# Banksylel/Restrictive-Hierarchical-Semantic-Segmentation

Measured on AMD Instinct MI355X. Metric: train images/sec (620x620, hier-HRNet-W48), higher is better.
Workload: dtype f32 (fp16x2 split on fp16 MFMA, 22-bit operands, fp32 accumulate; exact-fp32 MFMA on the small problems); 1 GPU; HRNet-W48 hierarchical (class_tree_tl.json), 620x620, batch 4 per GPU, train_epoch batch body (fwd L passes, prediction prep + metrics, CE+Dice+consistency, bwd, grad all-reduce, AdamW, metric vectors, one D2H readback of loss+metrics); global_batch=4, parallelism=dp1, launch=launch tape replay, rccl_ranks=1, level_passes=batched (one launch per layer for all L passes)

## Files before the change

### restrictive-hierarchical-semantic-segmentation_amd/Models/models.py

```python
from __future__ import annotations

import os

import torch
import torch.nn as nn

from .. import _lib, ops
from ..engine import Act, FlatParams, Recorder
from ..utils.hierarchy import build_hierarchy_indices, child_groups, get_level_classes

BN_MOMENTUM = 0.1
DEFAULT_CONV_DTYPE = "auto"


class Conv2d(nn.Conv2d):

    def forward(self, x):
        raise RuntimeError("hrseg_amd layers run inside the model's engine, not standalone")


class BatchNorm2d(nn.BatchNorm2d):
    def forward(self, x):
        raise RuntimeError("hrseg_amd layers run inside the model's engine, not standalone")

# ... 652 lines not shown
                                         nn.ReLU(inplace=True))
        final_k = extra["FINAL_CONV_KERNEL"]
        if final_k != 1:
            raise NotImplementedError("FINAL_CONV_KERNEL=3 heads are not built (the shipped W48 config uses 1)")
        if model_type == 0:
            n_leaves = sum(len(v) for v in get_level_classes(hierarchy, inc_parent=False).values())
            self.classifier = Conv2d(last, n_leaves, kernel_size=1, stride=1, padding=0)
        else:
            self.levels, self.parent_of, self.children_of = build_hierarchy_indices(hierarchy)
            self.child_groups = child_groups(self.levels, self.children_of)
            self.classifiers = nn.ModuleList([Conv2d(last, len(self.levels[0]), kernel_size=1)])
            for groups in self.child_groups:
                n = sum(len(ch) for _, ch in groups)
                self.classifiers.append(Conv2d(last, n if n > 0 else 1, kernel_size=1))
            self.films = nn.ModuleList([FiLM(feat_ch=last, cond_ch=len(self.levels[L - 1]))
                                        for L in range(1, len(self.levels))])
            if self.concat_prev_logits:
                _check_cond_stem_width([3 + self.classifiers[L - 1].out_channels for L in range(1, len(self.levels))])
                self.cond_stems = nn.ModuleList([Conv2d(3 + self.classifiers[L - 1].out_channels, 64, kernel_size=3, stride=2,
                                                        padding=1, bias=False) for L in range(1, len(self.levels))])
        self._init_engine()

    _make_layer = staticmethod(_make_layer)

    def _make_stage(self, layer_config, num_inchannels, multi_scale_output=True):
        block = blocks_dict[layer_config["BLOCK"]]
        modules = []
        for i in range(layer_config["NUM_MODULES"]):
            multi = multi_scale_output or i != layer_config["NUM_MODULES"] - 1
            modules.append(HighResolutionModule(layer_config["NUM_BRANCHES"], block, layer_config["NUM_BLOCKS"],
                                                num_inchannels, layer_config["NUM_CHANNELS"],
                                                layer_config.get("FUSE_METHOD"), multi, self.align_corners))
            num_inchannels = modules[-1].get_num_inchannels()
        return nn.Sequential(*modules), num_inchannels

    @staticmethod
    def _make_transition_layer(pre, cur):
        layers = []
        for i, c in enumerate(cur):
            if i < len(pre):
                if c != pre[i]:
                    layers.append(nn.Sequential(Conv2d(pre[i], c, 3, 1, 1, bias=False), _bn(c), nn.ReLU(inplace=True)))
                else:
                    layers.append(None)
            else:
                steps = []
                for j in range(i + 1 - len(pre)):
                    cout = c if j == i - len(pre) else pre[-1]
                    steps.append(nn.Sequential(Conv2d(pre[-1], cout, 3, 2, 1, bias=False), _bn(cout),
                                               nn.ReLU(inplace=True)))
                layers.append(nn.Sequential(*steps))
        return nn.ModuleList(layers)

    def _flat_head(self):
        return self.classifier

    def _level_head(self, L):
        return self.classifiers[L]

    def _backbone(self, rec, x, first=None):
        x = rec.conv_bn(x, first if first is not None else self.stem[0], self.stem[1], relu=True)
        x = rec.conv_bn(x, self.stem[3], self.stem[4], relu=True)
        rec.mark("layer1")
        x = _run_seq(rec, self.layer1, x)
        ys = [x]
        for t_idx in (1, 2, 3):
            rec.mark(f"transition{t_idx}")
            cfg = getattr(self, f"stage{t_idx + 1}_cfg")
            trans = getattr(self, f"transition{t_idx}")
            xs = []
            for i in range(cfg["NUM_BRANCHES"]):
                if trans[i] is None:
                    xs.append(ys[i])
                else:
                    src = ys[i] if i < len(ys) else ys[-1]
                    if isinstance(trans[i][0], nn.Sequential):
                        xs.append(_run_conv_chain(rec, trans[i], src))
                    else:
                        xs.append(rec.conv_bn(src, trans[i][0], trans[i][1], relu=True))
            ys = xs
            for mod in getattr(self, f"stage{t_idx + 1}"):
                ys = mod.run(rec, ys)
        rec.mark("shared_head")
        cat = rec.upsample_concat(ys, self.align_corners)
        return rec.conv_bn(cat, self.shared_head[0], self.shared_head[1], relu=True)

    def forward(self, x):
        return self._forward_impl(x)

    def init_weights(self, pretrained="", device="cpu"):
        checkpoint = torch.load(pretrained, map_location=device)
        if "state_dict" in checkpoint:
            checkpoint = checkpoint["state_dict"]
        stripped = {}
        for k, v in checkpoint.items():
            for prefix in ("model.", "module.", "net.", "network."):
                if k.startswith(prefix):
                    k = k[len(prefix):]
            stripped[k] = v
        own = self.state_dict()
        picked = {}
        for mk, mv in own.items():
            if mk in stripped and stripped[mk].size() == mv.size():
                picked[mk] = stripped[mk]
                continue
            for ck, cv in stripped.items():
                if (mk.endswith(ck) or ck.endswith(mk)) and cv.size() == mv.size():
                    picked[mk] = cv
                    break
        missing = set(own) - set(picked)
        print(f"Loaded {len(picked)} / {len(own)} layers.")
        if missing:
            print(f"Missing {len(missing)} layers (first 10): {list(missing)[:10]}")
        own.update(picked)
        self.load_state_dict(own)
        return self
```

### restrictive-hierarchical-semantic-segmentation_amd/csrc/bn_elem.hip

```cpp
#include "common.h"

struct Lanes {
  int Q, P, cq, pl;
  bool active;
};
__device__ __forceinline__ Lanes make_lanes(int C) {
  Lanes l;
  l.Q = C >> 2;
  l.P = (l.Q >= 256) ? 1 : 256 / l.Q;
  l.cq = threadIdx.x % l.Q;
  l.pl = threadIdx.x / l.Q;
  l.active = l.pl < l.P;
  return l;
}
static int elem_grid(long npix, int C) {
  const int Q = C / 4, P = (Q >= 256) ? 1 : 256 / Q;
  long blocks = (npix + P - 1) / P;
  if (blocks > 4096) blocks = 4096;
  if (blocks < 1) blocks = 1;
  return (int)blocks;
}
#define FOR_PIXELS(pix, L, npix) \
  for (long pix = (long)blockIdx.x * (L).P + (L).pl; pix < (npix); pix += (long)gridDim.x * (L).P)

// ... 261 lines not shown
                                                           int Hi, int Wi, int C) {
  const Lanes L = make_lanes(C);
  if (!L.active) return;
  const int Hc = (Hi + 1) / 2, Wc = (Wi + 1) / 2;
  const int Ho = Hi / 2, Wo = Wi / 2;
  const long ncell = (long)B * Hc * Wc;
  FOR_PIXELS(cell, L, ncell) {
    const int b = (int)(cell / ((long)Hc * Wc));
    const int rem = (int)(cell - (long)b * Hc * Wc);
    const int oy = rem / Wc, ox = rem - oy * Wc;
    const size_t base = (((size_t)b * Hi + 2 * oy) * Wi + 2 * ox);
    const bool full = (oy < Ho) & (ox < Wo);
    f32x4 g = {0.f, 0.f, 0.f, 0.f};
    int arg[4] = {-1, -1, -1, -1};
    if (full) {
      g = ld4(dy + (((size_t)b * Ho + oy) * Wo + ox) * lddy + 4 * L.cq);
      f32x4 m = ld4(x + base * ldx + 4 * L.cq);
#pragma unroll
      for (int j = 0; j < 4; ++j) arg[j] = 0;
#pragma unroll
      for (int k = 1; k < 4; ++k) {
        const f32x4 v = ld4(x + (base + (k >> 1) * Wi + (k & 1)) * ldx + 4 * L.cq);
#pragma unroll
        for (int j = 0; j < 4; ++j)
          if (v[j] > m[j]) { m[j] = v[j]; arg[j] = k; }
      }
    }
#pragma unroll
    for (int k = 0; k < 4; ++k) {
      const int iy = 2 * oy + (k >> 1), ix = 2 * ox + (k & 1);
      if (iy >= Hi || ix >= Wi) continue;
      f32x4 o;
#pragma unroll
      for (int j = 0; j < 4; ++j) o[j] = (arg[j] == k) ? g[j] : 0.f;
      float* d = dx + (base + (k >> 1) * Wi + (k & 1)) * lddx + 4 * L.cq;
      st4(d, acc ? ld4(d) + o : o);
    }
  }
}

__device__ __forceinline__ void src_index(int o, float scale, int in_size, int align, int& i0, int& i1,
                                          float& l0, float& l1) {
  float r;
  if (align) {
    r = scale * (float)o;
  } else {
    r = scale * ((float)o + 0.5f) - 0.5f;
    if (r < 0.f) r = 0.f;
  }
  i0 = (int)r;
  if (i0 > in_size - 1) i0 = in_size - 1;
  i1 = i0 + ((i0 < in_size - 1) ? 1 : 0);
  l1 = r - (float)i0;
  l0 = 1.f - l1;
}
static float resize_scale(int in_size, int out_size, int align) {
  if (align) return out_size > 1 ? (float)(in_size - 1) / (float)(out_size - 1) : 0.f;
  return (float)in_size / (float)out_size;
}

__global__ __launch_bounds__(256) void bilinear_fwd_kernel(const float* __restrict__ in, int ldin, int B, int Hi,
                                                           int Wi, int C, float* __restrict__ out, int ldout,
                                                           int Hout, int Wout, int Hr, int Wr, int py, int px,
                                                           float sh, float sw, int align, int acc, int relu) {
  const Lanes L = make_lanes(C);
  if (!L.active) return;
  const long npix = (long)B * Hout * Wout;
  FOR_PIXELS(pix, L, npix) {
    const int b = (int)(pix / ((long)Hout * Wout));
    const int rem = (int)(pix - (long)b * Hout * Wout);
    const int oy = rem / Wout - py, ox = rem % Wout - px;
    f32x4 v = {0.f, 0.f, 0.f, 0.f};
    if (oy >= 0 && oy < Hr && ox >= 0 && ox < Wr) {
      int y0, y1, x0, x1;
      float ly0, ly1, lx0, lx1;
      src_index(oy, sh, Hi, align, y0, y1, ly0, ly1);
      src_index(ox, sw, Wi, align, x0, x1, lx0, lx1);
      const float* p = in + (size_t)b * Hi * Wi * ldin + 4 * L.cq;
      const f32x4 v00 = ld4(p + ((size_t)y0 * Wi + x0) * ldin), v01 = ld4(p + ((size_t)y0 * Wi + x1) * ldin);
      const f32x4 v10 = ld4(p + ((size_t)y1 * Wi + x0) * ldin), v11 = ld4(p + ((size_t)y1 * Wi + x1) * ldin);
      v = ly0 * (lx0 * v00 + lx1 * v01) + ly1 * (lx0 * v10 + lx1 * v11);
    }
    float* o = out + pix * ldout + 4 * L.cq;
    if (acc) v += ld4(o);
    if (relu) {
#pragma unroll
      for (int j = 0; j < 4; ++j) v[j] = fmaxf(v[j], 0.f);
    }
    st4(o, v);
  }
}

struct FuseSumArgs {
  int n_same, n_low;
  const float* same[4]; int ld_same[4];
  const float* low[3]; int ld_low[3]; int Hi[3], Wi[3];
  float sh[3], sw[3];
  float* out; int ldo;
  int B, H, W, C, align, relu;
};
__global__ __launch_bounds__(256) void fuse_sum_kernel(FuseSumArgs a) {
  const Lanes L = make_lanes(a.C);
  if (!L.active) return;
  const long npix = (long)a.B * a.H * a.W;
  FOR_PIXELS(pix, L, npix) {
    f32x4 v = ld4(a.same[0] + pix * a.ld_same[0] + 4 * L.cq);
#pragma unroll
    for (int i = 1; i < 4; ++i)
      if (i < a.n_same) v += ld4(a.same[i] + pix * a.ld_same[i] + 4 * L.cq);
    if (a.n_low) {
      const int b = (int)(pix / ((long)a.H * a.W));
      const int rem = (int)(pix - (long)b * a.H * a.W);
      const int oy = rem / a.W, ox = rem - oy * a.W;
#pragma unroll
      for (int j = 0; j < 3; ++j)
        if (j < a.n_low) {
          int y0, y1, x0, x1;
          float ly0, ly1, lx0, lx1;
          src_index(oy, a.sh[j], a.Hi[j], a.align, y0, y1, ly0, ly1);
          src_index(ox, a.sw[j], a.Wi[j], a.align, x0, x1, lx0, lx1);
          const int ld = a.ld_low[j], Wi = a.Wi[j];
          const float* p = a.low[j] + (size_t)b * a.Hi[j] * Wi * ld + 4 * L.cq;
          const f32x4 v00 = ld4(p + ((size_t)y0 * Wi + x0) * ld), v01 = ld4(p + ((size_t)y0 * Wi + x1) * ld);
          const f32x4 v10 = ld4(p + ((size_t)y1 * Wi + x0) * ld), v11 = ld4(p + ((size_t)y1 * Wi + x1) * ld);
          v += ly0 * (lx0 * v00 + lx1 * v01) + ly1 * (lx0 * v10 + lx1 * v11);
        }
    }
    if (a.relu) {
#pragma unroll
      for (int j = 0; j < 4; ++j) v[j] = fmaxf(v[j], 0.f);
    }
    st4(a.out + pix * a.ldo + 4 * L.cq, v);
  }
}

template <int RS>
__global__ __launch_bounds__(256) void bilinear_bwd_kernel(const float* __restrict__ dout, int lddout, int B,
                                                           int Hi, int Wi, int C, float* __restrict__ din,
                                                           int lddin, int Hout, int Wout, int Hr, int Wr, int py,
                                                           int px, float sh, float sw, int align, int acc) {
  __shared__ f32x4 red[256];
  const int Q = C >> 2;
  const int P2 = max(1, 256 / (Q * RS));
  const int cq = threadIdx.x % Q, pl = (threadIdx.x / Q) % P2, rs = threadIdx.x / (Q * P2);
  const bool active = rs < RS && (int)threadIdx.x < Q * P2 * RS;
  const long npix = (long)B * Hi * Wi;
  const float ish = sh > 0.f ? 1.f / sh : 0.f, isw = sw > 0.f ? 1.f / sw : 0.f;
  for (long base = (long)blockIdx.x * P2; base < npix; base += (long)gridDim.x * P2) {
    const long pix = base + pl;
    f32x4 s = {0.f, 0.f, 0.f, 0.f};
    if (active && pix < npix) {
      const int b = (int)(pix / ((long)Hi * Wi));
      const int rem = (int)(pix - (long)b * Hi * Wi);
      const int iy = rem / Wi, ix = rem - iy * Wi;
      int oy_lo = 0, oy_hi = Hr - 1, ox_lo = 0, ox_hi = Wr - 1;
      if (sh > 0.f) {
        oy_lo = max(0, (int)floorf(((float)iy - 1.f + (align ? 0.f : 0.5f)) * ish - (align ? 0.f : 0.5f)) - 1);
        oy_hi = min(Hr - 1, (int)ceilf(((float)iy + 1.f + (align ? 0.f : 0.5f)) * ish - (align ? 0.f : 0.5f)) + 1);
      }
      if (sw > 0.f) {
        ox_lo = max(0, (int)floorf(((float)ix - 1.f + (align ? 0.f : 0.5f)) * isw - (align ? 0.f : 0.5f)) - 1);
        ox_hi = min(Wr - 1, (int)ceilf(((float)ix + 1.f + (align ? 0.f : 0.5f)) * isw - (align ? 0.f : 0.5f)) + 1);
      }
      for (int oy = oy_lo + rs; oy <= oy_hi; oy += RS) {
        int y0, y1;
        float ly0, ly1;
        src_index(oy, sh, Hi, align, y0, y1, ly0, ly1);
        const float wy = (y0 == iy ? ly0 : 0.f) + (y1 == iy ? ly1 : 0.f);
        if (wy == 0.f) continue;
        const float* row = dout + (((size_t)b * Hout + oy + py) * Wout + px) * lddout + 4 * cq;
        for (int ox = ox_lo; ox <= ox_hi; ++ox) {
          int x0, x1;
          float lx0, lx1;
          src_index(ox, sw, Wi, align, x0, x1, lx0, lx1);
          const float wx = (x0 == ix ? lx0 : 0.f) + (x1 == ix ? lx1 : 0.f);
          if (wx == 0.f) continue;
          s += (wy * wx) * ld4(row + (size_t)ox * lddout);
        }
      }
    }
    if (RS > 1) {
      __syncthreads();
      red[threadIdx.x] = s;
      __syncthreads();
      if (active && rs == 0) {
#pragma unroll
        for (int r = 1; r < RS; ++r) s += red[threadIdx.x + r * Q * P2];
      }
    }
    if (active && rs == 0 && pix < npix) {
      float* d = din + pix * lddin + 4 * cq;
      st4(d, acc ? ld4(d) + s : s);
    }
  }
}

__global__ __launch_bounds__(256) void add_kernel(const float* __restrict__ a, int lda, const float* __restrict__ b,
                                                  int ldb, float* __restrict__ out, int ldo, int relu, long npix,
                                                  int C) {
  const Lanes L = make_lanes(C);
  if (!L.active) return;
  FOR_PIXELS(pix, L, npix) {
    f32x4 v = ld4(a + pix * lda + 4 * L.cq) + ld4(b + pix * ldb + 4 * L.cq);
    if (relu) {
#pragma unroll
      for (int j = 0; j < 4; ++j) v[j] = fmaxf(v[j], 0.f);
    }
    st4(out + pix * ldo + 4 * L.cq, v);
  }
}
__global__ __launch_bounds__(256) void copy_kernel(const float* __restrict__ in, int ldin, float* __restrict__ out,
                                                   int ldout, int acc, long npix, int C) {
  const Lanes L = make_lanes(C);
  if (!L.active) return;
  FOR_PIXELS(pix, L, npix) {
    f32x4 v = ld4(in + pix * ldin + 4 * L.cq);
    float* o = out + pix * ldout + 4 * L.cq;
    st4(o, acc ? ld4(o) + v : v);
  }
}
__global__ __launch_bounds__(256) void relu_bwd_kernel(const float* __restrict__ dz, int lddz,
                                                       const float* __restrict__ z, int ldz, float* __restrict__ dx,
                                                       int lddx, long npix, int C) {
  const Lanes L = make_lanes(C);
  if (!L.active) return;
  FOR_PIXELS(pix, L, npix) {
    f32x4 g = ld4(dz + pix * lddz + 4 * L.cq);
    const f32x4 zz = ld4(z + pix * ldz + 4 * L.cq);
#pragma unroll
    for (int j = 0; j < 4; ++j) g[j] = zz[j] > 0.f ? g[j] : 0.f;
    st4(dx + pix * lddx + 4 * L.cq, g);
  }
}

__global__ __launch_bounds__(256) void absmax_kernel(const float* __restrict__ x, int ldx, long npix, int C,
                                                     float* __restrict__ out) {
  const Lanes L = make_lanes(C);
  float amax = 0.f;
  if (L.active) {
    FOR_PIXELS(pix, L, npix) {
      const f32x4 v = ld4(x + pix * ldx + 4 * L.cq);
#pragma unroll
      for (int j = 0; j < 4; ++j) amax = fmaxf(amax, (v[j] != v[j]) ? __builtin_inff() : fabsf(v[j]));
    }
  }
  __shared__ float wmax[4];
#pragma unroll
  for (int o = 32; o > 0; o >>= 1) amax = fmaxf(amax, __shfl_xor(amax, o, 64));
  if ((threadIdx.x & 63) == 0) wmax[threadIdx.x >> 6] = amax;
  __syncthreads();
  if (threadIdx.x == 0) {
    const float m = fmaxf(fmaxf(wmax[0], wmax[1]), fmaxf(wmax[2], wmax[3]));
    if (m > 0.f) atomicMax(reinterpret_cast<unsigned*>(out) + (blockIdx.x & 63), __float_as_uint(m));
  }
}

__global__ void nchw_to_nhwc_kernel(const float* __restrict__ in, float* __restrict__ out, int ldout, int B, int C,
                                    long hw) {
  const long i = (long)blockIdx.x * blockDim.x + threadIdx.x;
  if (i >= (long)B * hw) return;
  const long b = i / hw, p = i - b * hw;
  for (int c = 0; c < C; ++c) out[i * ldout + c] = in[(b * C + c) * hw + p];
}
__global__ void nhwc_to_nchw_kernel(const float* __restrict__ in, int ldin, float* __restrict__ out, int B, int C,
                                    long hw) {
  const long i = (long)blockIdx.x * blockDim.x + threadIdx.x;
  if (i >= (long)B * hw) return;
  const long b = i / hw, p = i - b * hw;
  for (int c = 0; c < C; ++c) out[(b * C + c) * hw + p] = in[i * ldin + c];
}

__global__ void fill_kernel(float* p, float v, long n) {
  for (long i = (long)blockIdx.x * blockDim.x + threadIdx.x; i < n; i += (long)gridDim.x * blockDim.x) p[i] = v;
}

__global__ __launch_bounds__(256) void adamw_kernel(float* __restrict__ p, const float* __restrict__ g,
                                                    float* __restrict__ m, float* __restrict__ v, long n4, long n,
                                                    float lr, float b1, float b2, float eps, float wd, float bc1,
                                                    float rsqrt_bc2, float gscale) {
  const float step = lr / bc1;
  for (long i = (long)blockIdx.x * blockDim.x + threadIdx.x; i < n4; i += (long)gridDim.x * blockDim.x) {
    f32x4 pp = ld4(p + 4 * i), gg = ld4(g + 4 * i) * gscale, mm = ld4(m + 4 * i), vv = ld4(v + 4 * i);
    pp = pp * (1.f - lr * wd);
    mm = mm + (gg - mm) * (1.f - b1);
    vv = vv * b2 + gg * gg * (1.f - b2);
#pragma unroll
    for (int j = 0; j < 4; ++j) pp[j] -= step * mm[j] / (sqrtf(vv[j]) * rsqrt_bc2 + eps);
    st4(p + 4 * i, pp);
    st4(m + 4 * i, mm);
    st4(v + 4 * i, vv);
  }
  if (blockIdx.x == 0 && threadIdx.x < (n - 4 * n4)) {
    const long i = 4 * n4 + threadIdx.x;
    float pp = p[i] * (1.f - lr * wd), gg = g[i] * gscale;
    const float mm = m[i] + (gg - m[i]) * (1.f - b1), vv = v[i] * b2 + gg * gg * (1.f - b2);
    p[i] = pp - step * mm / (sqrtf(vv) * rsqrt_bc2 + eps);
    m[i] = mm;
    v[i] = vv;
  }
}

// ... 336 lines not shown
  return 0;
}

extern "C" int hrseg_bn_eval_coef(const float* gamma, const float* beta, const float* running_mean,
                                  const float* running_var, float eps, int C, float* coef, hrseg_stream_t stream) {
  HRSEG_CHECK_ARG(running_mean && running_var && coef && C > 0, "hrseg_bn_eval_coef: bad arguments");
  hipLaunchKernelGGL(bn_eval_coef_kernel, dim3(ceil_div(C, 64)), dim3(64), 0, (hipStream_t)stream, gamma, beta,
                     running_mean, running_var, eps, C, coef);
  HRSEG_LAUNCH_CHECK("bn_eval_coef");
  return 0;
}

extern "C" int hrseg_bn_apply(const float* y, int ldy, const float* coef, const float* residual, int ldr, int relu,
                              float* z, int ldz, long npix, int C, hrseg_stream_t stream) {
  if (int e = check_c(C, "hrseg_bn_apply")) return e;
  HRSEG_CHECK_ARG(y && coef && z && npix > 0 && ldy >= C && ldz >= C && (ldy % 4 == 0) && (ldz % 4 == 0),
                  "hrseg_bn_apply: bad arguments");
  hipLaunchKernelGGL(bn_apply_kernel, dim3(elem_grid(npix, C)), dim3(256), 0, (hipStream_t)stream, y, ldy, coef,
                     residual, ldr, relu, z, ldz, npix, C);
  HRSEG_LAUNCH_CHECK("bn_apply");
  return 0;
}

extern "C" int hrseg_bn_bwd_reduce(const float* dz, int lddz, const float* z, int ldz, int relu, const float* y,
                                   int ldy, const float* coef, long npix, int C, double* partial, int nchunks,
                                   hrseg_stream_t stream) {
  if (int e = check_c(C, "hrseg_bn_bwd_reduce")) return e;
  HRSEG_CHECK_ARG(dz && y && coef && partial && (!relu || z) && npix > 0 && nchunks > 0,
                  "hrseg_bn_bwd_reduce: bad arguments");
  hipLaunchKernelGGL(bn_bwd_reduce_kernel, dim3(nchunks), dim3(256), 0, (hipStream_t)stream, dz, lddz, z, ldz, relu, y,
                     ldy, coef, npix, C, partial, chunk_size(npix, nchunks));
  HRSEG_LAUNCH_CHECK("bn_bwd_reduce");
  return 0;
}

extern "C" int hrseg_bn_bwd_apply(const double* partial, int nchunks, const float* dz, int lddz, const float* z,
                                  int ldz, int relu, const float* y, int ldy, const float* coef, const float* gamma,
                                  float* dgamma, float* dbeta, float* dy, int lddy, float* dres, int lddres,
                                  int dres_accumulate, long npix, int C, int eval_mode, hrseg_stream_t stream) {
  if (int e = check_c(C, "hrseg_bn_bwd_apply")) return e;
  (void)gamma;
  HRSEG_CHECK_ARG(partial && dz && y && coef && dy && (!relu || z) && npix > 0 && nchunks > 0,
                  "hrseg_bn_bwd_apply: bad arguments");
  hipStream_t st = (hipStream_t)stream;
  double* totals = (double*)partial + (size_t)nchunks * 2 * C;
  hipLaunchKernelGGL(bn_bwd_finalize_kernel, dim3(ceil_div(C, 16)), dim3(256), 0, st, partial, totals, nchunks, C,
                     dgamma, dbeta);
  HRSEG_LAUNCH_CHECK("bn_bwd_finalize");
  hipLaunchKernelGGL(bn_bwd_apply_kernel, dim3(elem_grid(npix, C)), dim3(256), 0, st, totals, dz, lddz, z, ldz, relu,
                     y, ldy, coef, dy, lddy, dres, lddres, dres_accumulate, npix, C, eval_mode);
  HRSEG_LAUNCH_CHECK("bn_bwd_apply");
  return 0;
}

extern "C" int hrseg_maxpool2_fwd(const float* x, int ldx, float* y, int ldy, int B, int Hi, int Wi, int C,
                                  hrseg_stream_t stream) {
  if (int e = check_c(C, "hrseg_maxpool2_fwd")) return e;
  HRSEG_CHECK_ARG(x && y && B > 0 && Hi >= 2 && Wi >= 2, "hrseg_maxpool2_fwd: bad arguments");
  const long npix = (long)B * (Hi / 2) * (Wi / 2);
  hipLaunchKernelGGL(maxpool2_fwd_kernel, dim3(elem_grid(npix, C)), dim3(256), 0, (hipStream_t)stream, x, ldx, y, ldy,
                     B, Hi, Wi, C);
  HRSEG_LAUNCH_CHECK("maxpool2_fwd");
  return 0;
}

extern "C" int hrseg_maxpool2_bwd(const float* x, int ldx, const float* dy, int lddy, float* dx, int lddx,
                                  int accumulate, int B, int Hi, int Wi, int C, hrseg_stream_t stream) {
  if (int e = check_c(C, "hrseg_maxpool2_bwd")) return e;
  HRSEG_CHECK_ARG(x && dy && dx && B > 0 && Hi >= 2 && Wi >= 2, "hrseg_maxpool2_bwd: bad arguments");
  const long ncell = (long)B * ((Hi + 1) / 2) * ((Wi + 1) / 2);
  hipLaunchKernelGGL(maxpool2_bwd_kernel, dim3(elem_grid(ncell, C)), dim3(256), 0, (hipStream_t)stream, x, ldx, dy,
                     lddy, dx, lddx, accumulate, B, Hi, Wi, C);
  HRSEG_LAUNCH_CHECK("maxpool2_bwd");
  return 0;
}

extern "C" int hrseg_bilinear_fwd(const float* in, int ldin, int B, int Hi, int Wi, int C, float* out, int ldout,
                                  int Hout, int Wout, int Hr, int Wr, int py, int px, int align_corners,
                                  int accumulate, int relu, hrseg_stream_t stream) {
  if (int e = check_c(C, "hrseg_bilinear_fwd")) return e;
  HRSEG_CHECK_ARG(in && out && B > 0 && Hi > 0 && Wi > 0 && Hr > 0 && Wr > 0 && py >= 0 && px >= 0 &&
                      py + Hr <= Hout && px + Wr <= Wout,
                  "hrseg_bilinear_fwd: placed image %dx%d at (%d,%d) does not fit %dx%d", Hr, Wr, py, px, Hout, Wout);
  const long npix = (long)B * Hout * Wout;
  hipLaunchKernelGGL(bilinear_fwd_kernel, dim3(elem_grid(npix, C)), dim3(256), 0, (hipStream_t)stream, in, ldin, B, Hi,
                     Wi, C, out, ldout, Hout, Wout, Hr, Wr, py, px, resize_scale(Hi, Hr, align_corners),
                     resize_scale(Wi, Wr, align_corners), align_corners, accumulate, relu);
  HRSEG_LAUNCH_CHECK("bilinear_fwd");
  return 0;
}

extern "C" int hrseg_bilinear_bwd(const float* dout, int lddout, int B, int Hi, int Wi, int C, float* din, int lddin,
                                  int Hout, int Wout, int Hr, int Wr, int py, int px, int align_corners,
                                  int accumulate, hrseg_stream_t stream) {
  if (int e = check_c(C, "hrseg_bilinear_bwd")) return e;
  HRSEG_CHECK_ARG(dout && din && B > 0 && Hi > 0 && Wi > 0 && Hr > 0 && Wr > 0 && py >= 0 && px >= 0 &&
                      py + Hr <= Hout && px + Wr <= Wout,
                  "hrseg_bilinear_bwd: bad geometry");
  const long npix = (long)B * Hi * Wi;
  const int Q = C / 4;
  const int foot = (Hi > 1 && Hr > 1) ? (int)(2.0 * (Hr - 1) / (Hi - 1)) + 3 : Hr;
  int rs = 1;
  while (rs < 8 && Q * rs * 2 <= 256 && rs * 2 <= foot / 2 && npix / max(1, 256 / (Q * rs)) < 1024) rs *= 2;
  const int P2 = max(1, 256 / (Q * rs));
  long blocks = (npix + P2 - 1) / P2;
  if (blocks > 4096) blocks = 4096;
  const float sh = resize_scale(Hi, Hr, align_corners), sw = resize_scale(Wi, Wr, align_corners);
#define HRSEG_BIL(RS_) hipLaunchKernelGGL(bilinear_bwd_kernel<RS_>, dim3((unsigned)blocks), dim3(256), 0, (hipStream_t)stream, \
                                          dout, lddout, B, Hi, Wi, C, din, lddin, Hout, Wout, Hr, Wr, py, px, sh, sw,         \
                                          align_corners, accumulate)
  if (rs == 1) HRSEG_BIL(1); else if (rs == 2) HRSEG_BIL(2); else if (rs == 4) HRSEG_BIL(4); else HRSEG_BIL(8);
#undef HRSEG_BIL
  HRSEG_LAUNCH_CHECK("bilinear_bwd");
  return 0;
}

extern "C" int hrseg_fuse_sum(int n_same, const float* const* same, const int* ld_same, int n_low, const float* const* low,
                              const int* ld_low, const int* Hi, const int* Wi, float* out, int ldo, int B, int H, int W, int C,
                              int align_corners, int relu, hrseg_stream_t stream) {
  if (int e = check_c(C, "hrseg_fuse_sum")) return e;
  HRSEG_CHECK_ARG(n_same >= 1 && n_same <= 4 && n_low >= 0 && n_low <= 3 && same && ld_same && out && B > 0 && H > 0 && W > 0,
                  "hrseg_fuse_sum: 1..4 same-resolution terms and 0..3 low-resolution terms");
  HRSEG_CHECK_ARG(n_low == 0 || (low && ld_low && Hi && Wi), "hrseg_fuse_sum: low-resolution terms need their geometry");
  FuseSumArgs a{};
  a.n_same = n_same; a.n_low = n_low;
  for (int i = 0; i < n_same; ++i) {
    HRSEG_CHECK_ARG(same[i] && ld_same[i] >= C && ld_same[i] % 4 == 0, "hrseg_fuse_sum: bad same-resolution term %d", i);
    a.same[i] = same[i]; a.ld_same[i] = ld_same[i];
  }
  for (int j = 0; j < n_low; ++j) {
    HRSEG_CHECK_ARG(low[j] && ld_low[j] >= C && ld_low[j] % 4 == 0 && Hi[j] > 0 && Wi[j] > 0, "hrseg_fuse_sum: bad low-resolution term %d", j);
    a.low[j] = low[j]; a.ld_low[j] = ld_low[j]; a.Hi[j] = Hi[j]; a.Wi[j] = Wi[j];
    a.sh[j] = resize_scale(Hi[j], H, align_corners);
    a.sw[j] = resize_scale(Wi[j], W, align_corners);
  }
  a.out = out; a.ldo = ldo; a.B = B; a.H = H; a.W = W; a.C = C; a.align = align_corners; a.relu = relu;
  const long npix = (long)B * H * W;
  hipLaunchKernelGGL(fuse_sum_kernel, dim3(elem_grid(npix, C)), dim3(256), 0, (hipStream_t)stream, a);
  HRSEG_LAUNCH_CHECK("fuse_sum");
  return 0;
}

extern "C" int hrseg_add(const float* a, int lda, const float* b, int ldb, float* out, int ldo, int relu, long npix,
                         int C, hrseg_stream_t stream) {
  if (int e = check_c(C, "hrseg_add")) return e;
  HRSEG_CHECK_ARG(a && b && out && npix > 0, "hrseg_add: bad arguments");
  hipLaunchKernelGGL(add_kernel, dim3(elem_grid(npix, C)), dim3(256), 0, (hipStream_t)stream, a, lda, b, ldb, out, ldo,
                     relu, npix, C);
  HRSEG_LAUNCH_CHECK("add");
  return 0;
}

extern "C" int hrseg_copy(const float* in, int ldin, float* out, int ldout, int accumulate, long npix, int C,
                          hrseg_stream_t stream) {
  if (int e = check_c(C, "hrseg_copy")) return e;
  HRSEG_CHECK_ARG(in && out && npix > 0, "hrseg_copy: bad arguments");
  hipLaunchKernelGGL(copy_kernel, dim3(elem_grid(npix, C)), dim3(256), 0, (hipStream_t)stream, in, ldin, out, ldout,
                     accumulate, npix, C);
  HRSEG_LAUNCH_CHECK("copy");
  return 0;
}

extern "C" int hrseg_relu_bwd(const float* dz, int lddz, const float* z, int ldz, float* dx, int lddx, long npix,
                              int C, hrseg_stream_t stream) {
  if (int e = check_c(C, "hrseg_relu_bwd")) return e;
  HRSEG_CHECK_ARG(dz && z && dx && npix > 0, "hrseg_relu_bwd: bad arguments");
  hipLaunchKernelGGL(relu_bwd_kernel, dim3(elem_grid(npix, C)), dim3(256), 0, (hipStream_t)stream, dz, lddz, z, ldz,
                     dx, lddx, npix, C);
  HRSEG_LAUNCH_CHECK("relu_bwd");
  return 0;
}

extern "C" int hrseg_absmax(const float* x, int ldx, long npix, int C, float* out64, hrseg_stream_t stream) {
  if (int e = check_c(C, "hrseg_absmax")) return e;
  HRSEG_CHECK_ARG(x && out64 && npix > 0 && ldx >= C, "hrseg_absmax: bad arguments");
  hipLaunchKernelGGL(absmax_kernel, dim3(elem_grid(npix, C)), dim3(256), 0, (hipStream_t)stream, x, ldx, npix, C, out64);
  HRSEG_LAUNCH_CHECK("absmax");
  return 0;
}

extern "C" int hrseg_nchw_to_nhwc(const float* in, float* out, int ldout, int B, int C, int H, int W,
                                  hrseg_stream_t stream) {
  HRSEG_CHECK_ARG(in && out && B > 0 && C > 0 && ldout >= C, "hrseg_nchw_to_nhwc: bad arguments");
  const long n = (long)B * H * W;
  hipLaunchKernelGGL(nchw_to_nhwc_kernel, dim3(ceil_div(n, 256)), dim3(256), 0, (hipStream_t)stream, in, out, ldout, B,
                     C, (long)H * W);
  HRSEG_LAUNCH_CHECK("nchw_to_nhwc");
  return 0;
}

extern "C" int hrseg_nhwc_to_nchw(const float* in, int ldin, float* out, int B, int C, int H, int W,
                                  hrseg_stream_t stream) {
  HRSEG_CHECK_ARG(in && out && B > 0 && C > 0 && ldin >= C, "hrseg_nhwc_to_nchw: bad arguments");
  const long n = (long)B * H * W;
  hipLaunchKernelGGL(nhwc_to_nchw_kernel, dim3(ceil_div(n, 256)), dim3(256), 0, (hipStream_t)stream, in, ldin, out, B,
                     C, (long)H * W);
  HRSEG_LAUNCH_CHECK("nhwc_to_nchw");
  return 0;
}

extern "C" int hrseg_fill(float* p, float v, long n, hrseg_stream_t stream) {
  HRSEG_CHECK_ARG(p && n >= 0, "hrseg_fill: bad arguments");
  if (n == 0) return 0;
  long blocks = (n + 255) / 256;
  if (blocks > 4096) blocks = 4096;
  hipLaunchKernelGGL(fill_kernel, dim3((int)blocks), dim3(256), 0, (hipStream_t)stream, p, v, n);
  HRSEG_LAUNCH_CHECK("fill");
  return 0;
}

extern "C" int hrseg_adamw(float* p, const float* g, float* m, float* v, long n, float lr, float beta1, float beta2,
                           float eps, float weight_decay, float bc1, float bc2, float gscale,
                           hrseg_stream_t stream) {
  HRSEG_CHECK_ARG(p && g && m && v && n > 0, "hrseg_adamw: bad arguments");
  HRSEG_CHECK_ARG(((uintptr_t)p % 16 == 0) && ((uintptr_t)g % 16 == 0) && ((uintptr_t)m % 16 == 0) &&
                      ((uintptr_t)v % 16 == 0),
                  "hrseg_adamw: buffers must be 16-byte aligned");
  const long n4 = n / 4;
  long blocks = (n4 + 255) / 256;
  if (blocks > 8192) blocks = 8192;
  if (blocks < 1) blocks = 1;
  hipLaunchKernelGGL(adamw_kernel, dim3((int)blocks), dim3(256), 0, (hipStream_t)stream, p, g, m, v, n4, n, lr, beta1,
                     beta2, eps, weight_decay, bc1, 1.0f / sqrtf(bc2), gscale);
  HRSEG_LAUNCH_CHECK("adamw");
  return 0;
}

extern "C" int hrseg_adamw_dev(float* p, const float* g, float* m, float* v, long n, const float* hyper, float* state,
                               hrseg_stream_t stream) {
  HRSEG_CHECK_ARG(p && g && m && v && hyper && state && n > 0, "hrseg_adamw_dev: bad arguments");
  HRSEG_CHECK_ARG(((uintptr_t)p % 16 == 0) && ((uintptr_t)g % 16 == 0) && ((uintptr_t)m % 16 == 0) &&
                      ((uintptr_t)v % 16 == 0),
                  "hrseg_adamw_dev: buffers must be 16-byte aligned");
  hipStream_t st = (hipStream_t)stream;
  hipLaunchKernelGGL(adam_tick_kernel, dim3(1), dim3(64), 0, st, state, hyper);
  HRSEG_LAUNCH_CHECK("adam_tick");
  const long n4 = n / 4;
  long blocks = (n4 + 255) / 256;
  if (blocks > 8192) blocks = 8192;
// ... 99 lines not shown
```

### restrictive-hierarchical-semantic-segmentation_amd/csrc/conv.hip

```cpp
#include "conv_common.h"
#include "conv_sp.h"
#include <mutex>
#include <vector>

enum { CNT_WS = 0, CNT_WS_GROUP, CNT_PATCH_SP, CNT_SP_IM2COL, CNT_SP_PGROUP, CNT_SP_GROUP, CNT_F32, CNT_F32_GROUP, CNT_WGRAD_SP,
       CNT_WGRAD_F32, CNT_WGRAD_F32_GROUP, CNT_WGRAD9, CNT_SMALL_CIN, CNT_SP_WIDE, CNT_WS_CANVAS, CNT_WGRAD_SP_GROUP, CNT_WGRAD_SP_T5, CNT_WGRAD_SP_WIDE, CNT_AUG_IMAGE, CNT_AUG_TARGETS, CNT_N };
static const char* const g_cnt_names[CNT_N] = {"ws", "ws_group", "patch_sp", "sp_im2col", "sp_pgroup", "sp_group", "f32", "f32_group",
                                               "wgrad_sp", "wgrad_f32", "wgrad_f32_group", "wgrad9", "small_cin", "sp_wide", "ws_canvas", "wgrad_sp_group", "wgrad_sp_t5", "wgrad_sp_wide",
                                               "augment_image", "augment_targets"};
static long g_cnt[CNT_N];
static bool in_conv_total(int i) { return i != CNT_WS_CANVAS && i != CNT_WGRAD_SP_T5 && i != CNT_AUG_IMAGE && i != CNT_AUG_TARGETS; }
extern "C" long hrseg_launch_count(const char* family, int reset) {
  long total = 0;
  for (int i = 0; i < CNT_N; ++i)
    if (family ? !strcmp(family, g_cnt_names[i]) : in_conv_total(i)) { total += g_cnt[i]; if (reset) g_cnt[i] = 0; }
  if (!family && reset)
    for (int i = 0; i < CNT_N; ++i) g_cnt[i] = 0;
  return total;
}
void hrseg_count_augment_launches(int image, int targets) {
  g_cnt[CNT_AUG_IMAGE] += image;
  g_cnt[CNT_AUG_TARGETS] += targets;
}

// ... 326 lines not shown
  if (a.stat_partial) *a.stat_rows = (int)grid.x;
  ++g_cnt[CNT_WS];
  g_cnt[CNT_WS_CANVAS] += a.cv_w1 > 0;
  return launch_ws_kernel(a, kind, flip, (int)grid.x, ntotal, st, ns);
}
static int launch_ws_group(IgemmArgs* a, const int* kinds, int n, hipStream_t st, int ns = 4) {
  IgemmGroup g;
  g.n = n;
  long cost[MAXG], ntot[MAXG], total = 0;
  int blocks[MAXG], flip = -1;
  for (int i = 0; i < n; ++i) {
    if (a[i].x_presplit && ns != 4) return 1;
    const int f = patch_flip(a[i]);
    if (flip >= 0 && f != flip) return 1;
    flip = f;
    const int cs = WS_CS[kinds[i]];
    ws_set_canvas(a[i], kinds[i]);
    ntot[i] = ws_tiles(a[i], kinds[i]);
    a[i].epi_early = g_ws_epi_early;
    a[i].exp_nosplit = (g_exp_nosplit && !f) ? 1 : 0;
    const int ec = g_ws_epi_cost ? (g_ws_epi_cost > 0 ? g_ws_epi_cost : 0) : WS_EPI_COST;
    const int eac = g_ws_epi_acc_cost ? (g_ws_epi_acc_cost > 0 ? g_ws_epi_acc_cost : 0) : WS_EPI_ACC_COST;
    cost[i] = (long)(a[i].K / (16 * cs)) * ((9 * cs + 1) / 2) + ((a[i].accumulate || a[i].res) ? eac : ec);
    total += ntot[i] * cost[i];
  }
  int used = 0;
  for (int i = 0; i < n; ++i) {
    blocks[i] = (int)(256 * ntot[i] * cost[i] / total);
    if (blocks[i] < 1) blocks[i] = 1;
    if (blocks[i] > ntot[i]) blocks[i] = (int)ntot[i];
    used += blocks[i];
  }
  auto span = [&](int i, int b) { return (long)ceil_div((int)ntot[i], b) * cost[i]; };
  for (int it = 0; it < 512; ++it) {
    int hi = 0, lo = -1;
    for (int i = 1; i < n; ++i)
      if (span(i, blocks[i]) > span(hi, blocks[hi])) hi = i;
    if (blocks[hi] >= ntot[hi]) break;
    if (used < 256) { ++blocks[hi]; ++used; continue; }
    for (int i = 0; i < n; ++i)
      if (i != hi && blocks[i] > 1 && (lo < 0 || span(i, blocks[i] - 1) < span(lo, blocks[lo] - 1))) lo = i;
    if (lo < 0 || span(lo, blocks[lo] - 1) >= span(hi, blocks[hi])) break;
    --blocks[lo];
    ++blocks[hi];
  }
  if (!ws_make_images(a, kinds, n, st, ns)) return 1;
  int end = 0;
  for (int i = 0; i < n; ++i) {
    const int per = ceil_div((int)ntot[i], blocks[i]);
    g.tiles[i] = ceil_div((int)ntot[i], per);
    if (a[i].stat_partial) *a[i].stat_rows = g.tiles[i];
    g.ksplit[i] = (int)ntot[i];
    end += g.tiles[i];
    g.blk_end[i] = end;
    g.kind[i] = kinds[i];
    g.a[i] = a[i];
    g_cnt[CNT_WS_CANVAS] += a[i].cv_w1 > 0;
  }
  ++g_cnt[CNT_WS_GROUP];
  return launch_ws_group_kernel(g, flip, st, ns);
}

static int g_sp_img = 1;
static int g_sp_persist = 2;
static int launch_patch_sp(int ns, const IgemmArgs& a_in, int wtn, int cs, hipStream_t st) {
  const int ntotal = (int)patch_tiles(a_in, wtn);
  int blocks = ntotal;
  if (g_sp_persist > 0 && ntotal > 256 * g_sp_persist) {
    const int per = ceil_div(ntotal, 256 * g_sp_persist);
    blocks = ceil_div(ntotal, per);
  }
  const int flip = patch_flip(a_in);
  IgemmArgs a = a_in;
  if (ns == 4 && g_sp_img) {
    int kind = (wtn == 3 && cs == 3) ? 1 : (wtn == 6 && cs == 3) ? 2 : (wtn == 4 && cs == 4) ? 3 : 0;
    if (kind) ws_make_images(&a, &kind, 1, st, 4);
  }
  ++g_cnt[CNT_PATCH_SP];
  return launch_patch_sp_kernel(ns, a, wtn, cs, flip, blocks, ntotal, st);
}

static int g_sp_wide = 1;
static int g_spw_min_blocks = 256;
static int spw_wtn(const IgemmArgs& a) {
  if (!g_sp_wide || !scratch_usable() || a.K % 16 || a.M < 128) return 0;
  const int wtn = (a.N % 240 == 0) ? 15 : (a.N % 192 == 0) ? 12 : (a.N % 128 == 0) ? 8 : (a.N % 96 == 0) ? 6 : 0;
  if (!wtn) return 0;
  if ((long)ceil_div(a.M, 128) * (a.N / (16 * wtn)) < g_spw_min_blocks) return 0;
  const int nslabs = (a.ntaps * (a.K / 16) + 1) / 2, padded = (nslabs + 5) / 6 * 6;
  if (g_sp_wide < 2 && (padded - nslabs) * 10 > nslabs) return 0;
  return wtn;
}

static int launch_sp(int ns, const IgemmArgs& a, const SpPlan& pl, hipStream_t st) {
  if (launch_sp_kernel(ns, a, pl, st) == 0) { ++g_cnt[CNT_SP_IM2COL]; return 0; }
  hrseg_set_error("igemm_sp: no kernel for plan wtm=%d wtn=%d", pl.wtm, pl.wtn);
  return HRSEG_ERR_UNSUPPORTED;
}

static int sp_pieces(int precision) {
  return precision == HRSEG_CONV_BF16X3 ? 3 : precision == HRSEG_CONV_BF16X2 ? 2 : precision == HRSEG_CONV_BF16 ? 1
       : precision == HRSEG_CONV_FP16X2 ? 4 : 0;
}
static bool is_f16(int precision) { return precision == HRSEG_CONV_FP16X2 || precision == HRSEG_CONV_AUTO; }
static void set_sp_scales(IgemmArgs& a, int precision, const float* grad_absmax) {
  const bool f16 = is_f16(precision);
  a.wscale = f16 ? 256.f : 1.f;
  a.wscale_inv = f16 ? 1.f / 256.f : 1.f;
  a.xmax = f16 ? grad_absmax : nullptr;
}

static int resolve_auto(const IgemmArgs& a, int precision) {
  if (precision != HRSEG_CONV_AUTO) return precision;
  if (a.M >= g_auto_min_pix) return HRSEG_CONV_FP16X2;
  const int k = ws_kind(a);
  return (k && ws_tiles(a, k) >= g_ws_min_tiles) ? HRSEG_CONV_FP16X2 : HRSEG_CONV_F32;
}

static int x_split_unsupported(const char* who) {
  hrseg_set_error("%s: x_split is set but this problem does not run the wave-specialised / nine-tap kernels (ask hrseg_conv_x_split_ok first)", who);
  return HRSEG_ERR_UNSUPPORTED;
}
static int dispatch_igemm(const IgemmArgs& a_in, int precision, hipStream_t st) {
  IgemmArgs a = a_in;
  if (int e = finalize_args(a)) return e;
  precision = resolve_auto(a, precision);
  if (const int ns = sp_pieces(precision)) {
    const SpPlan pl = plan_sp(a);
    if ((ns == 4 || (ns == 1 && g_ws_bf16)) && !g_sp_wtn) {
      const int kind = ws_kind(a);
      if (kind && ws_tiles(a, kind) >= g_ws_min_tiles && launch_ws_single(a, kind, st, ns) == 0) return 0;
    }
    if (a.x_presplit) return x_split_unsupported("hrseg_conv_fwd");
    if (const int cs = patch_cs(a, pl.wtn)) {
      const int rc = launch_patch_sp(ns, a, pl.wtn, cs, st);
      if (rc == 0) return 0;
    }
    if (ns == 4 && !g_sp_wtn) {
      const int wtn = spw_wtn(a);
      if (wtn) {
        const size_t bytes = (size_t)(a.N / (16 * wtn)) * ((a.ntaps * (a.K / 16) + 1) / 2) * (size_t)(2 * 16 * wtn * 64);
        if (unsigned char* img = scratch_reserve(st, bytes)) {
          ++g_cnt[CNT_SP_WIDE];
          if (launch_spw_kernel(a, wtn, 1, img, st) == 0) return 0;
        }
      }
    }
    if (pl.ksplit > 1 && !a.accumulate) zero_f32(a.y, (size_t)a.B * a.Hy * a.Wy * a.N, st);
    return launch_sp(ns, a, pl, st);
  }
  if (a.x_presplit) return x_split_unsupported("hrseg_conv_fwd");
  IgemmPlan pl = plan_igemm(a);
  if (pl.ksplit > 1 && !a.accumulate) zero_f32(a.y, (size_t)a.B * a.Hy * a.Wy * a.N, st);
  if (launch_igemm_f32(a, pl, st) == 0) { ++g_cnt[CNT_F32]; return 0; }
  hrseg_set_error("igemm: no kernel for plan wtm=%d wtn=%d kc=%d db=%d", pl.wtm, pl.wtn, pl.kc, pl.db);
  return HRSEG_ERR_UNSUPPORTED;
}

static int g_group_wtm = 0;

static int launch_sp_group(int ns, const IgemmGroup& g_in, int wtm, int wtn, int cs, hipStream_t st) {
  IgemmGroup g = g_in;
  if (ns == 4 && cs && g_sp_img && ((wtn == 3 && cs == 3) || (wtn == 4 && cs == 4))) {
    IgemmArgs im[MAXG];
    int kinds[MAXG], idx[MAXG], m = 0;
    for (int i = 0; i < g.n; ++i)
      if (g.kind[i]) { im[m] = g.a[i]; kinds[m] = wtn == 3 ? 1 : 3; idx[m++] = i; }
    if (m && ws_make_images(im, kinds, m, st, 4))
      for (int j = 0; j < m; ++j) g.a[idx[j]].wimg = im[j].wimg;
  }
  bool full = true;
  for (int i = 0; i < g.n; ++i) full = full && g.a[i].ntaps == 9 && g.a[i].T == 9 && g.a[i].sy == 1 && g.a[i].oys == 1;
  if (cs) {
    int flip = -1;
    for (int i = 0; i < g.n; ++i)
      if (g.kind[i]) {
        const int f = patch_flip(g.a[i]);
        if (flip >= 0 && f != flip) return 1;
        flip = f;
      }
    ++g_cnt[CNT_SP_PGROUP];
    return launch_sp_pgroup_kernel(ns, g, wtm, wtn, cs, flip, st);
  }
  ++g_cnt[CNT_SP_GROUP];
  return launch_sp_group_kernel(ns, g, wtm, wtn, full, st);
}

static int dispatch_igemm_group(const IgemmArgs* a, int n, int precision, hipStream_t st);
static int dispatch_igemm_group_auto(const IgemmArgs* a, int n, hipStream_t st, bool try_ws = true) {
  if (try_ws && g_sp_ws && scratch_usable() && !g_sp_wtn) {
    IgemmArgs wsa[MAXG], rest[MAXG];
    int kinds[MAXG], nw = 0, nr = 0;
    for (int i = 0; i < n; ++i) {
      IgemmArgs f = a[i];
      if (finalize_args(f)) return 1;
      const int k = ws_kind(f);
      if (k && ws_tiles(f, k) >= g_ws_min_tiles) { wsa[nw] = f; kinds[nw++] = k; }
      else rest[nr++] = a[i];
    }
    bool pair = false;
    if (nw == 1 && nr == 1) {
      IgemmArgs f = rest[0];
      pair = finalize_args(f) == 0 && f.N % 48 == 0 && patch_cs(f, 3) == 3;
    }
    bool split_rest = false;
    for (int i = 0; i < nr; ++i) split_rest = split_rest || rest[i].x_presplit;
    if (split_rest || (pair && (wsa[0].x_presplit))) return x_split_unsupported("hrseg_conv_fwd_group");
    if (nw >= 1 && !pair && launch_ws_group(wsa, kinds, nw, st) == 0) {
      if (nr == 0) return 0;
      if (nr == 1) { const int e = dispatch_igemm(rest[0], HRSEG_CONV_AUTO, st); return e < 0 ? e : (e ? HRSEG_ERR_LAUNCH : 0); }
      if (dispatch_igemm_group_auto(rest, nr, st, false) == 0) return 0;
      for (int i = 0; i < nr; ++i)
        if (int e = dispatch_igemm(rest[i], HRSEG_CONV_AUTO, st)) return e < 0 ? e : HRSEG_ERR_LAUNCH;
      return 0;
    }
  }
  for (int i = 0; i < n; ++i)
    if (a[i].x_presplit) return x_split_unsupported("hrseg_conv_fwd_group");
  IgemmArgs hi[MAXG], lo[MAXG];
  int nh = 0, nl = 0;
  for (int i = 0; i < n; ++i) {
    IgemmArgs f = a[i];
    if (finalize_args(f)) return 1;
    const int wtn = (f.N % 48 == 0) ? 3 : (f.N % 64 == 0) ? 4 : 0;
    if (wtn && patch_cs(f, wtn) == wtn) hi[nh++] = a[i];
    else lo[nl++] = a[i];
  }
  if (nh == 0) {
    bool small = true, large = true;
    for (int i = 0; i < n; ++i) { small = small && a[i].M < g_auto_min_pix; large = large && a[i].M >= g_auto_min_pix; }
// ... 42 lines not shown
  int wtn = (a[0].N % 48 == 0) ? 3 : (a[0].N % 64 == 0) ? 4 : 0;
  const int kc = ns ? 1 : (a[0].K % 48 == 0) ? 3 : (a[0].K % 32 == 0) ? 2 : 1;
  if (!wtn) return 1;
  if (ns && g_sp_wtn) {
    bool ok = true;
    for (int i = 0; i < n; ++i) ok = ok && a[i].N % (16 * g_sp_wtn) == 0;
    if (ok && (g_sp_wtn == 3 || g_sp_wtn == 4 || g_sp_wtn == 6)) wtn = g_sp_wtn;
  }
  IgemmGroup g;
  g.n = n;
  for (int i = 0; i < n; ++i)
    if (a[i].N % (16 * wtn) || a[i].K % (16 * kc)) return 1;
  int tiles[MAXG], ks[MAXG], work[MAXG], order[MAXG], kind[MAXG];
  const int wtm = ns ? (g_sp_wtm ? g_sp_wtm : 2) : (g_group_wtm ? g_group_wtm : 1);
  if (ns && wtm > 2) return 1;
  int group_cs = 0;
  IgemmArgs fa[MAXG];
  for (int i = 0; i < n; ++i) {
    fa[i] = a[i];
    if (finalize_args(fa[i])) return 1;
    kind[i] = 0;
    if (ns && (wtn == 3 || wtn == 4)) {
      const int cs = patch_cs(fa[i], wtn);
      if (cs && cs == wtn && (!group_cs || group_cs == cs)) { kind[i] = 1; group_cs = cs; }
    }
  }
  for (int i = 0; i < n; ++i) {
    tiles[i] = kind[i] ? (int)patch_tiles(fa[i], wtn) : ceil_div(a[i].M, 64 * wtm) * (a[i].N / (16 * wtn));
    const int nstages = ns ? (a[i].ntaps * (a[i].K / 16) + 1) / 2 : a[i].ntaps * (a[i].K / (16 * kc));
    ks[i] = 1;
    const bool can_split = !kind[i] && !a[i].res && !a[i].relu &&
                           (a[i].accumulate || (a[i].ldy == a[i].N && a[i].oys == 1 && a[i].oxs == 1));
    if (can_split && tiles[i] < 512 && !hrseg_g_deterministic) {
      ks[i] = ceil_div(512, tiles[i]);
      const int min_stages = ns ? 8 : 12;
      if (ks[i] > nstages / min_stages) ks[i] = nstages / min_stages;
      if (ks[i] < 1) ks[i] = 1;
    }
    if (ks[i] > 1 && !a[i].accumulate) zero_f32(a[i].y, (size_t)a[i].B * a[i].Hy * a[i].Wy * a[i].N, st);
    work[i] = ceil_div(nstages, ks[i]);
    order[i] = i;
  }
  for (int i = 0; i < n; ++i)
    for (int j = i + 1; j < n; ++j)
      if (work[order[j]] > work[order[i]]) { const int t = order[i]; order[i] = order[j]; order[j] = t; }
  int end = 0;
  for (int o = 0; o < n; ++o) {
    const int i = order[o];
    g.tiles[o] = tiles[i];
    g.ksplit[o] = ks[i];
    end += tiles[i] * ks[i];
    g.blk_end[o] = end;
    g.kind[o] = kind[i];
    g.a[o] = fa[i];
  }
  if (ns) return launch_sp_group(ns, g, wtm, wtn, group_cs, st);
  ++g_cnt[CNT_F32_GROUP];
  return launch_igemm_group_f32(g, wtm, wtn, kc, st);
}

static int g_tune_wg_pix = 0, g_tune_wg_db = 0, g_tune_wg_blocks = 0;

int check_wgrad_span(const WgradArgs& a) {
  const double imgs = (double)ceil_div(a.pix_per_block, a.Ho * a.Wo) + 1.0;
  if (imgs * a.Hi * a.Wi * (double)a.ldx * 4.0 >= 4294967296.0 || (double)a.pix_per_block * a.lddy * 4.0 >= 4294967296.0) {
    hrseg_set_error("wgrad: a block's pixel range (%d pixels) exceeds the 4 GB buffer-offset range", a.pix_per_block);
    return HRSEG_ERR_UNSUPPORTED;
  }
  return 0;
}

static int g_wg_t5 = 1;
static int g_wg_wide = 1;
static int ksplit_for_rounds(int tiles, int kmin, int kmax, int slots) {
  int best = 0;
  double best_eff = 0.0;
  for (int k = kmin; k <= kmax; ++k) {
    const int blocks = tiles * k;
    const double eff = (double)blocks / (ceil_div(blocks, slots) * (double)slots);
    if (eff > best_eff + 1e-9) { best_eff = eff; best = k; }
  }
  return best;
}
static int dispatch_wgrad_sp(int ns, WgradArgs a, hipStream_t st) {
  if (ns == 4 && g_wg_wide && a.Cout % 240 == 0 && a.Cin % 144 == 0 && a.M >= 65536 && !hrseg_g_deterministic && !g_tune_wg_blocks) {
    const int tiles = (a.Cout / 240) * (a.Cin / 144) * a.T;
    int kmax = a.M / 2048;
    if (kmax > 64) kmax = 64;
    const int ksplit = ksplit_for_rounds(tiles, 1, kmax, 256);
    a.pix_per_block = ceil_div(ceil_div(a.M, ksplit), 32) * 32;
    if (int e = check_wgrad_span(a)) return e;
    ++g_cnt[CNT_WGRAD_SP_WIDE];
    return launch_wgrad_spw_kernel(a, ceil_div(a.M, a.pix_per_block), tiles, st);
  }
  int tn = (a.Cout % 48 == 0) ? 3 : (a.Cout % 64 == 0) ? 4 : (a.Cout % 32 == 0) ? 2 : 1;
  int tk = (a.Cin % 48 == 0) ? 3 : (a.Cin % 64 == 0) ? 4 : (a.Cin % 32 == 0) ? 2 : 1;
  constexpr int PIX = 128;
  const bool t5 = ns == 4 && g_wg_t5 && a.Cout % 80 == 0 && a.Cin % 80 == 0 && (long)a.Cout * a.Cin >= 240 * 240 && a.M >= 65536;
  if (t5) tn = tk = 5;
  const int tiles = (a.Cout / (16 * tn)) * (a.Cin / (16 * tk)) * a.T;
  int target = 7 * tiles;
  if (target < 512) target = 512;
  if (target > 4096) target = 4096;
  if (t5) {
    int kmax = a.M / (PIX * 8);
    if (kmax > 32) kmax = 32;
    if (const int best = ksplit_for_rounds(tiles, 4, kmax, 256)) target = best * tiles;
  }
  if (g_tune_wg_blocks) target = g_tune_wg_blocks;
  int ksplit = target / tiles;
  if (ksplit < 1 || hrseg_g_deterministic) ksplit = 1;
  int ppb = ceil_div(ceil_div(a.M, ksplit), PIX) * PIX;
  if (ppb < 2 * PIX) ppb = 2 * PIX;
  a.pix_per_block = ppb;
  if (int e = check_wgrad_span(a)) return e;
  const int gx = ceil_div(a.M, ppb);
  ++g_cnt[CNT_WGRAD_SP];
  g_cnt[CNT_WGRAD_SP_T5] += t5;
  return launch_wgrad_sp_kernel(ns, a, tn, tk, gx, tiles, st);
}

static int g_wg_mult = 0, g_wg_min = 0, g_wg_max = 0;
static void plan_wgrad_blocks(WgradArgs& a, int tn, int tk, int pix, int& gx, int& tiles) {
  tiles = (a.Cout / (16 * tn)) * (a.Cin / (16 * tk)) * a.T;
  int target = (g_wg_mult ? g_wg_mult : 2) * tiles;
  const int tmin = g_wg_min ? g_wg_min : 768, tmax = g_wg_max ? g_wg_max : 2048;
  if (target < tmin) target = tmin;
  if (target > tmax) target = tmax;
  int ksplit = target / tiles;
  if (ksplit < 1 || hrseg_g_deterministic) ksplit = 1;
  int ppb = ceil_div(ceil_div(a.M, ksplit), pix) * pix;
  if (ppb < 4 * pix) ppb = 4 * pix;
  a.pix_per_block = ppb;
  gx = ceil_div(a.M, ppb);
}

static int g_wg_group_sp = 1;
static int dispatch_wgrad_group(WgradArgs* a, int n, int prec, hipStream_t st) {
  if (n < 2 || n > MAXG || g_tune_wg_pix || g_tune_wg_db || g_tune_wg_blocks) return 1;
  const bool sp = prec == HRSEG_CONV_FP16X2 && g_wg_group_sp;
  const int tn = (a[0].Cout % 48 == 0) ? 3 : (a[0].Cout % 64 == 0) ? 4 : 0;
  const int tk = (a[0].Cin % 48 == 0) ? 3 : (a[0].Cin % 64 == 0) ? 4 : 0;
  if (!tn || !tk) return 1;
  WgradGroup g;
  g.n = n;
  int end = 0;
  for (int i = 0; i < n; ++i) {
    if (a[i].Cout % (16 * tn) || a[i].Cin % (16 * tk)) return 1;
    int gx, tiles;
    plan_wgrad_blocks(a[i], tn, tk, sp ? 128 : 64, gx, tiles);
    if (check_wgrad_span(a[i])) return 1;
    g.gx[i] = gx;
    end += gx * tiles;
    g.blk_end[i] = end;
    g.a[i] = a[i];
  }
  if (sp) {
    ++g_cnt[CNT_WGRAD_SP_GROUP];
    return launch_wgrad_group_sp(g, tn, tk, end, st);
  }
  ++g_cnt[CNT_WGRAD_F32_GROUP];
  return launch_wgrad_group_f32(g, tn, tk, end, st);
}

static int g_wg9_blocks = 0;
static int g_wg9_blocks_n[WG9_MAXG + 1] = {0, 0, 0, 0, 0};
static int g_wg9 = 1;
static int wgrad9_tnk(const hrseg_conv_shape_t& s) {
// ... 199 lines not shown
    if (int e = check_shape(&shapes[i], "hrseg_conv_fwd_group")) return e;
    ok = ok && mfma_shape(&shapes[i]) && shapes[i].precision == shapes[0].precision;
  }
  if (ok && n >= 2) {
    IgemmArgs a[MAXG];
    for (int i = 0; i < n; ++i) fill_fwd_args(a[i], x[i], w[i], bias ? bias[i] : nullptr, y[i], &shapes[i]);
    const int rc = dispatch_igemm_group(a, n, shapes[0].precision, st);
    if (rc < 0) return rc;
    if (rc == 0) {
      HRSEG_LAUNCH_CHECK("igemm_group(fwd)");
      return 0;
    }
  }
  for (int i = 0; i < n; ++i)
    if (int e = hrseg_conv_fwd(x[i], w[i], bias ? bias[i] : nullptr, y[i], &shapes[i], stream)) return e;
  return 0;
}

extern "C" int hrseg_conv_dgrad_group(int n, const float* const* dy, const float* const* wt, float* const* dx,
                                      const int* accumulate, const hrseg_conv_shape_t* shapes,
                                      hrseg_stream_t stream) {
  HRSEG_CHECK_ARG(n >= 1 && dy && wt && dx && accumulate && shapes, "hrseg_conv_dgrad_group: bad arguments");
  hipStream_t st = (hipStream_t)stream;
  bool ok = n <= MAXG;
  for (int i = 0; i < n; ++i) {
    if (int e = check_shape(&shapes[i], "hrseg_conv_dgrad_group")) return e;
    ok = ok && mfma_shape(&shapes[i]) && shapes[i].stride == 1 && shapes[i].precision == shapes[0].precision;
  }
  if (ok && n >= 2) {
    IgemmArgs a[MAXG];
    for (int i = 0; i < n; ++i) fill_dgrad_s1_args(a[i], dy[i], wt[i], dx[i], accumulate[i], &shapes[i]);
    const int rc = dispatch_igemm_group(a, n, shapes[0].precision, st);
    if (rc < 0) return rc;
    if (rc == 0) {
      HRSEG_LAUNCH_CHECK("igemm_group(dgrad)");
      return 0;
    }
  }
  for (int i = 0; i < n; ++i)
    if (int e = hrseg_conv_dgrad(dy[i], wt[i], dx[i], accumulate[i], &shapes[i], stream)) return e;
  return 0;
}

extern "C" int hrseg_conv_wgrad_group(int n, const float* const* x, const float* const* dy, float* const* dw,
                                      const hrseg_conv_shape_t* shapes, hrseg_stream_t stream) {
  HRSEG_CHECK_ARG(n >= 1 && x && dy && dw && shapes, "hrseg_conv_wgrad_group: bad arguments");
  for (int i = 0; i < n; ++i)
    if (shapes[i].x_split) return x_split_unsupported("hrseg_conv_wgrad_group");
  hipStream_t st = (hipStream_t)stream;
  bool ok = n <= MAXG;
  for (int i = 0; i < n; ++i) {
    if (int e = check_shape(&shapes[i], "hrseg_conv_wgrad_group")) return e;
    ok = ok && mfma_shape(&shapes[i]);
  }
  if (ok && n >= 2) {
    WgradArgs a[MAXG];
    hrseg_conv_shape_t rs[MAXG];
    resolve_wgrad_shapes(n, shapes, rs);
    int prec = rs[0].precision;
    for (int i = 0; i < n; ++i) {
      fill_wgrad_args(a[i], x[i], dy[i], dw[i], &rs[i]);
      if (rs[i].precision != prec) prec = HRSEG_CONV_F32;
    }
    if (dispatch_wgrad_group(a, n, prec, st) == 0) {
      HRSEG_LAUNCH_CHECK("wgrad_group");
      return 0;
    }
  }
  for (int i = 0; i < n; ++i)
    if (int e = hrseg_conv_wgrad(x[i], dy[i], dw[i], &shapes[i], stream)) return e;
  return 0;
}

extern "C" size_t hrseg_conv_wgrad_workspace_bytes(int n, const hrseg_conv_shape_t* shapes_in) {
  if (!shapes_in || n < 1 || n > WG9_MAXG) return 0;
  hrseg_conv_shape_t shapes[WG9_MAXG];
  resolve_wgrad_shapes(n, shapes_in, shapes);
  for (int i = 0; i < n; ++i)
    if (check_shape(&shapes[i], "hrseg_conv_wgrad_workspace_bytes")) return 0;
  return wgrad9_ws_bytes(n, shapes);
}

static int g_x_split = 1;
extern "C" int hrseg_conv_x_split_ok(int n, const hrseg_conv_shape_t* shapes) {
  if (!g_x_split || !shapes || n < 1 || n > MAXG || n > WG9_MAXG) return 0;
  if (!g_sp_ws || !scratch_usable() || g_sp_wtn || g_tune_wtm || g_tune_kc || g_tune_db || g_tune_ksplit) return 0;
  for (int i = 0; i < n; ++i) {
    const hrseg_conv_shape_t& s = shapes[i];
    if (s.ksize != 3 || s.stride != 1 || s.residual || s.relu || !mfma_shape(&s) || s.precision != shapes[0].precision) return 0;
    if (s.precision != HRSEG_CONV_AUTO && !(s.precision == HRSEG_CONV_FP16X2 && n == 1)) return 0;
    if (s.B < 1 || s.Hi < 1 || s.Wi < 1 || s.Ho != s.Hi || s.Wo != s.Wi) return 0;
    IgemmArgs a;
    fill_fwd_args(a, reinterpret_cast<const float*>(256), reinterpret_cast<const float*>(256), nullptr, reinterpret_cast<float*>(256), &s);
    a.stat_partial = nullptr; a.stat_rows = nullptr;
    if (finalize_args(a)) return 0;
    const int k = ws_kind(a);
    if (!k || ws_tiles(a, k) < g_ws_min_tiles) return 0;
  }
  hrseg_conv_shape_t rs[WG9_MAXG];
  resolve_wgrad_shapes(n, shapes, rs);
  for (int i = 0; i < n; ++i)
    if (sp_pieces(rs[i].precision) != 4) return 0;
  return wgrad9_ws_bytes(n, rs) > 0 ? 1 : 0;
}

extern "C" int hrseg_conv_wgrad_group_ws(int n, const float* const* x, const float* const* dy, float* const* dw,
                                         const hrseg_conv_shape_t* shapes_in, void* workspace, size_t workspace_bytes,
                                         hrseg_stream_t stream) {
  HRSEG_CHECK_ARG(n >= 1 && x && dy && dw && shapes_in, "hrseg_conv_wgrad_group_ws: bad arguments");
  if (n > WG9_MAXG) return hrseg_conv_wgrad_group(n, x, dy, dw, shapes_in, stream);
  hrseg_conv_shape_t shapes[WG9_MAXG];
  resolve_wgrad_shapes(n, shapes_in, shapes);
  for (int i = 0; i < n; ++i)
    if (int e = check_shape(&shapes[i], "hrseg_conv_wgrad_group_ws")) return e;
  const size_t need = wgrad9_ws_bytes(n, shapes);
  if (need && workspace && workspace_bytes >= need) {
    for (int i = 0; i < n; ++i) HRSEG_CHECK_ARG(x[i] && dy[i] && dw[i], "hrseg_conv_wgrad_group_ws: null pointer");
    return dispatch_wgrad9(n, x, dy, dw, shapes, (float*)workspace, (hipStream_t)stream);
  }
  return hrseg_conv_wgrad_group(n, x, dy, dw, shapes, stream);
}

extern "C" int hrseg_conv_fwd(const float* x, const float* w, const float* bias, float* y,
                              const hrseg_conv_shape_t* s, hrseg_stream_t stream) {
  if (int e = check_shape(s, "hrseg_conv_fwd")) return e;
  HRSEG_CHECK_ARG(x && w && y, "hrseg_conv_fwd: null pointer");
  hipStream_t st = (hipStream_t)stream;
  HRSEG_CHECK_ARG(s->Cout % 16 == 0 || s->Cin <= HRSEG_SMALL_CIN_MAX, "hrseg_conv_fwd: Cout %d not a multiple of 16", s->Cout);
  if (s->Cin <= HRSEG_SMALL_CIN_MAX) {
    launch_small_cin_fwd(x, w, bias, y, s, st);
    ++g_cnt[CNT_SMALL_CIN];
    HRSEG_LAUNCH_CHECK("conv_small_cin_fwd");
    return 0;
  }
  HRSEG_CHECK_ARG(s->Cin % 16 == 0, "hrseg_conv_fwd: Cin %d not a multiple of 16", s->Cin);
  HRSEG_CHECK_ARG(s->ldx % 4 == 0 && s->ldy % 4 == 0, "hrseg_conv_fwd: ld must be a multiple of 4");
  IgemmArgs a;
  fill_fwd_args(a, x, w, bias, y, s);
  if (int e = dispatch_igemm(a, s->precision, st)) return e;
  HRSEG_LAUNCH_CHECK("igemm_conv(fwd)");
  return 0;
}

extern "C" int hrseg_conv_dgrad(const float* dy, const float* wt, float* dx, int accumulate,
                                const hrseg_conv_shape_t* s, hrseg_stream_t stream) {
  if (int e = check_shape(s, "hrseg_conv_dgrad")) return e;
  HRSEG_CHECK_ARG(dy && wt && dx, "hrseg_conv_dgrad: null pointer");
  if (s->Cin <= HRSEG_SMALL_CIN_MAX) {
    launch_small_cin_dgrad(dy, wt, dx, accumulate, s, (hipStream_t)stream);
    ++g_cnt[CNT_SMALL_CIN];
    HRSEG_LAUNCH_CHECK("conv_small_cin_dgrad");
    return 0;
  }
  HRSEG_CHECK_ARG(s->Cin % 16 == 0 && s->Cout % 16 == 0, "hrseg_conv_dgrad: channels (%d,%d) must be multiples of 16",
                  s->Cin, s->Cout);
  HRSEG_CHECK_ARG(s->ldx % 4 == 0 && s->ldy % 4 == 0, "hrseg_conv_dgrad: ld must be a multiple of 4");
  hipStream_t st = (hipStream_t)stream;
  IgemmArgs a{};
  a.x = dy; a.w = wt; a.bias = nullptr; a.y = dx; a.ldx = s->ldy; a.ldy = s->ldx;
  a.B = s->B; a.Hi = s->Ho; a.Wi = s->Wo; a.K = s->Cout;
  a.N = s->Cin; a.T = s->ksize * s->ksize; a.accumulate = accumulate;
  a.Hy = s->Hi; a.Wy = s->Wi;
  set_sp_scales(a, s->precision, s->grad_absmax);
  const int ks = s->ksize, pad = (ks - 1) / 2;
  if (s->stride == 1) {
    a.Ho = s->Hi; a.Wo = s->Wi; a.M = s->B * s->Hi * s->Wi;
    a.sy = a.sx = 1; a.oys = a.oxs = 1; a.oy0 = a.ox0 = 0;
    int oy[9], ox[9], wtp[9];
    for (int t = 0; t < a.T; ++t) { oy[t] = pad - t / ks; ox[t] = pad - t % ks; wtp[t] = t; }
    pack_taps(a, a.T, oy, ox, wtp);
    if (int e = dispatch_igemm(a, s->precision, st)) return e;
    HRSEG_LAUNCH_CHECK("igemm_conv(dgrad)");
    return 0;
  }
  IgemmArgs cls[4];
  int ncls = 0;
  for (int py = 0; py < 2; ++py)
    for (int px = 0; px < 2; ++px) {
      const int hc = (s->Hi - py + 1) / 2, wc = (s->Wi - px + 1) / 2;
      if (hc <= 0 || wc <= 0) continue;
      int oy[9], ox[9], wtp[9], n = 0;
      for (int kh = 0; kh < ks; ++kh)
        for (int kw = 0; kw < ks; ++kw) {
          if (((py + pad - kh) & 1) || ((px + pad - kw) & 1)) continue;
          oy[n] = (py + pad - kh) >> 1;
          ox[n] = (px + pad - kw) >> 1;
          wtp[n] = kh * ks + kw;
          ++n;
        }
      IgemmArgs c = a;
      c.Ho = hc; c.Wo = wc; c.M = s->B * hc * wc;
      c.sy = c.sx = 1; c.oys = c.oxs = 2; c.oy0 = py; c.ox0 = px;
      pack_taps(c, n, oy, ox, wtp);
      cls[ncls++] = c;
    }
  if (ncls >= 2) {
    const int rc = dispatch_igemm_group(cls, ncls, s->precision, st);
    if (rc < 0) return rc;
    if (rc == 0) {
      HRSEG_LAUNCH_CHECK("igemm_group(dgrad s2)");
      return 0;
    }
  }
  for (int i = 0; i < ncls; ++i) {
    if (int e = dispatch_igemm(cls[i], s->precision, st)) return e;
    HRSEG_LAUNCH_CHECK("igemm_conv(dgrad s2)");
  }
  return 0;
}

extern "C" int hrseg_conv_wgrad(const float* x, const float* dy, float* dw, const hrseg_conv_shape_t* s_in,
                                hrseg_stream_t stream) {
  if (s_in && s_in->x_split) return x_split_unsupported("hrseg_conv_wgrad");
  HRSEG_CHECK_ARG(s_in != nullptr, "hrseg_conv_wgrad: null shape");
  hrseg_conv_shape_t sh;
  resolve_wgrad_shapes(1, s_in, &sh);
  const hrseg_conv_shape_t* s = &sh;
  if (int e = check_shape(s, "hrseg_conv_wgrad")) return e;
  HRSEG_CHECK_ARG(x && dy && dw, "hrseg_conv_wgrad: null pointer");
  hipStream_t st = (hipStream_t)stream;
  const int T = s->ksize * s->ksize;
  if (s->Cin <= HRSEG_SMALL_CIN_MAX) {
    const long M = (long)s->B * s->Ho * s->Wo;
    const int nblk_target = hrseg_g_deterministic ? 1 : g_tune_wg_blocks ? g_tune_wg_blocks : 512;
    int ppb = (int)ceil_div(ceil_div(M, nblk_target), 64) * 64;
    launch_small_cin_wgrad(x, dy, dw, s, ppb, st);
    ++g_cnt[CNT_SMALL_CIN];
    HRSEG_LAUNCH_CHECK("conv_small_cin_wgrad");
    return 0;
  }
  HRSEG_CHECK_ARG(s->Cin % 16 == 0 && s->Cout % 16 == 0, "hrseg_conv_wgrad: channels (%d,%d) must be multiples of 16",
                  s->Cin, s->Cout);
  HRSEG_CHECK_ARG(s->ldx % 4 == 0 && s->ldy % 4 == 0, "hrseg_conv_wgrad: ld must be a multiple of 4");
  WgradArgs a{};
  a.x = x; a.dy = dy; a.dw = dw; a.ldx = s->ldx; a.lddy = s->ldy;
  a.B = s->B; a.Hi = s->Hi; a.Wi = s->Wi; a.Cin = s->Cin; a.Ho = s->Ho; a.Wo = s->Wo; a.Cout = s->Cout;
  a.M = s->B * s->Ho * s->Wo; a.ks = s->ksize; a.stride = s->stride; a.T = T;
  const bool big = (long)s->B * s->Ho * s->Wo >= (1L << 24);
  a.rcp_hw = big ? 0.f : 1.0f / (float)(s->Ho * s->Wo);
  a.rcp_w = big ? 0.f : 1.0f / (float)s->Wo;
  a.dymax = s->precision == HRSEG_CONV_FP16X2 ? s->grad_absmax : nullptr;
  if (const int ns = sp_pieces(s->precision)) {
    if (int e = dispatch_wgrad_sp(ns, a, st)) return e;
    HRSEG_LAUNCH_CHECK("wgrad_sp");
    return 0;
  }
  const int tn = (s->Cout % 48 == 0) ? 3 : (s->Cout % 64 == 0) ? 4 : (s->Cout % 32 == 0) ? 2 : 1;
  const int tk = (s->Cin % 48 == 0) ? 3 : (s->Cin % 64 == 0) ? 4 : (s->Cin % 32 == 0) ? 2 : 1;
  {
    const int tiles = (a.Cout / (16 * tn)) * (a.Cin / (16 * tk)) * a.T;
    int pix = 64, db = 1, target = 7 * tiles;
    if (target < 512) target = 512;
    if (target > 4096) target = 4096;
    if (g_tune_wg_pix) pix = g_tune_wg_pix;
    if (g_tune_wg_db) db = g_tune_wg_db;
    if (g_tune_wg_blocks) target = g_tune_wg_blocks;
    if (int e = launch_wgrad_f32(a, tn, tk, pix, db, target, st)) return e;
    ++g_cnt[CNT_WGRAD_F32];
  }
  HRSEG_LAUNCH_CHECK("wgrad");
  return 0;
}

extern "C" int hrseg_weight_transpose(const float* w, float* wt, int Cout, int taps, int Cin,
                                      hrseg_stream_t stream) {
  HRSEG_CHECK_ARG(w && wt && Cout > 0 && taps > 0 && Cin > 0, "hrseg_weight_transpose: bad arguments");
  dim3 grid(ceil_div(Cin, 32), ceil_div(Cout, 32), taps);
  hipLaunchKernelGGL(weight_transpose_kernel, grid, dim3(32, 8), 0, (hipStream_t)stream, w, wt, Cout, taps, Cin);
  HRSEG_LAUNCH_CHECK("weight_transpose");
  return 0;
}

extern "C" int hrseg_weight_transpose_all(const float* flat, float* flat_t, const int* table, int nentries,
                                          hrseg_stream_t stream) {
  HRSEG_CHECK_ARG(flat && flat_t && table && nentries > 0, "hrseg_weight_transpose_all: bad arguments");
  hipLaunchKernelGGL(weight_transpose_all_kernel, dim3(nentries), dim3(32, 8), 0, (hipStream_t)stream, flat, flat_t,
                     table);
  HRSEG_LAUNCH_CHECK("weight_transpose_all");
  return 0;
}

extern "C" int hrseg_tune(const char* key, int value) {
  struct { const char* k; int* v; } tab[] = {
      {"igemm_wtm", &g_tune_wtm}, {"igemm_kc", &g_tune_kc}, {"igemm_db", &g_tune_db}, {"igemm_ksplit", &g_tune_ksplit},
      {"group_wtm", &g_group_wtm}, {"wgrad_pix", &g_tune_wg_pix}, {"wgrad_db", &g_tune_wg_db},
      {"wgrad_blocks", &g_tune_wg_blocks}, {"wgrad_group_mult", &g_wg_mult}, {"wgrad_group_min", &g_wg_min},
      {"wgrad_group_max", &g_wg_max}, {"sp_wtm", &g_sp_wtm}, {"sp_wtn", &g_sp_wtn}, {"sp_ksplit", &g_sp_ksplit}, {"sp_patch", &g_sp_patch}, {"sp_persist", &g_sp_persist}, {"sp_ws", &g_sp_ws}, {"sp_ws_waste", &g_ws_waste}, {"small_cin3", &g_small_cin3}, {"sp_ws_bf16", &g_ws_bf16}, {"sp_ws_n48", &g_ws_n48}, {"sp_img", &g_sp_img}, {"wgrad9", &g_wg9}, {"ws_epi_early", &g_ws_epi_early}, {"exp_nosplit_x", &g_exp_nosplit}, {"x_split", &g_x_split}, {"ws_epi_cost", &g_ws_epi_cost}, {"ws_epi_acc_cost", &g_ws_epi_acc_cost}, {"wgrad9_blocks", &g_wg9_blocks}, {"wgrad9_blocks1", &g_wg9_blocks_n[1]}, {"wgrad9_blocks2", &g_wg9_blocks_n[2]}, {"wgrad9_blocks3", &g_wg9_blocks_n[3]}, {"wgrad9_blocks4", &g_wg9_blocks_n[4]}, {"sp_wide", &g_sp_wide}, {"sp_ws_canvas", &g_ws_canvas}, {"wgrad_group_sp", &g_wg_group_sp}, {"wgrad_sp_t5", &g_wg_t5}, {"wgrad_sp_wide", &g_wg_wide}, {"sp_wide_min_blocks", &g_spw_min_blocks},
      {"sp_patch_min_tiles", &g_patch_min_tiles}, {"auto_min_pixels", &g_auto_min_pix}, {"sp_ws_min_tiles", &g_ws_min_tiles},
      {"deterministic", &hrseg_g_deterministic}};
  HRSEG_CHECK_ARG(key != nullptr, "hrseg_tune: null key");
  for (auto& e : tab)
    if (!strcmp(e.k, key)) {
      *e.v = value;
      if (g_patch_min_tiles <= 0) g_patch_min_tiles = 192;
      if (g_auto_min_pix <= 0) g_auto_min_pix = 8192;
      if (g_ws_min_tiles <= 0) g_ws_min_tiles = 96;
      return 0;
    }
  hrseg_set_error("hrseg_tune: unknown key '%s'", key);
  return HRSEG_ERR_INVALID_ARG;
}
```

### restrictive-hierarchical-semantic-segmentation_amd/csrc/conv_common.h

```cpp
#pragma once
#include "common.h"
#include <string.h>
#include <stdint.h>

struct IgemmArgs {
  const float* x;
  const float* w;
  const float* bias;
  float* y;
  int ldx, ldy;
  int B, Hi, Wi, K;
  int Ho, Wo, N;
  int M;
  int sy, sx;
  int Hy, Wy, oys, oxs, oy0, ox0;
  int ntaps;
  unsigned long long offy_pk, offx_pk, wtap_pk;
  int T;
  int accumulate;
  float rcp_hw, rcp_w;
  int direct_out;
  const float* xmax;
  float wscale, wscale_inv;
  int oy_min, ox_min;
  const unsigned char* wimg;
  int cv_w1, cv_nb;
  unsigned cv_magic;
  const float* res;
  int ldr, relu;
  int epi_early;
  double* stat_partial;
  int* stat_rows;
  int w_persistent;
  int exp_nosplit;
  int x_presplit;
};

__device__ __forceinline__ int fdiv(int n, int d, float rcp) {
  if (rcp <= 0.f) return n / d;
  int q = (int)((float)n * rcp);
  const int r = n - q * d;
  q += (r >= d) ? 1 : 0;
  q -= (r < 0) ? 1 : 0;
  return q;
}

typedef int i32x4_t __attribute__((ext_vector_type(4)));
typedef unsigned u32x4_t __attribute__((ext_vector_type(4)));
#define HRSEG_BUF_FLAGS 0x00020000
#define HRSEG_BUF_OOB 0xFFFFFFFFu
__device__ __forceinline__ __amdgpu_buffer_rsrc_t make_rsrc(const float* base, size_t bytes) {
  return __builtin_amdgcn_make_buffer_rsrc(const_cast<float*>(base), 0,
                                           (int)(bytes > 0xFFFFFFFFull ? 0xFFFFFFFFull : bytes), HRSEG_BUF_FLAGS);
}
__device__ __forceinline__ f32x4 buf_load4(__amdgpu_buffer_rsrc_t r, unsigned voff, int soff_bytes) {
  return __builtin_bit_cast(f32x4, __builtin_amdgcn_raw_buffer_load_b128(r, (int)voff, soff_bytes, 0));
}
__device__ __forceinline__ void buf_store4(__amdgpu_buffer_rsrc_t r, unsigned voff, int soff_bytes, const f32x4& v) {
  __builtin_amdgcn_raw_buffer_store_b128(__builtin_bit_cast(u32x4_t, v), r, (int)voff, soff_bytes, 0);
}

__device__ __forceinline__ int lds_slot(int row, int slot) { return slot ^ ((-(row >> 2)) & 3); }


#define MAXG 8
struct IgemmGroup {
  int n;
  int blk_end[MAXG];
  int tiles[MAXG];
  int ksplit[MAXG];
  int kind[MAXG];
  IgemmArgs a[MAXG];
};
struct WgradArgs {
  const float* x;
  const float* dy;
  float* dw;
  int ldx, lddy;
  int B, Hi, Wi, Cin, Ho, Wo, Cout;
  int M;
  int ks, stride, T;
  int pix_per_block;
  float rcp_hw, rcp_w;
  const float* dymax;
};

struct WgradGroup {
  int n;
  int blk_end[MAXG];
  int gx[MAXG];
  WgradArgs a[MAXG];
};
struct IgemmPlan { int wtm, wtn, kc, db, ksplit; };
struct SpPlan { int wtm, wtn, ksplit; };

int launch_igemm_f32(const IgemmArgs& a, const IgemmPlan& pl, hipStream_t st);
int launch_igemm_group_f32(const IgemmGroup& g, int wtm, int wtn, int kc, hipStream_t st);
int launch_wgrad_f32(const WgradArgs& a, int tn, int tk, int pix, int db, int target, hipStream_t st);
int launch_wgrad_group_f32(const WgradGroup& g, int tn, int tk, int nblocks, hipStream_t st);
int launch_sp_kernel(int ns, const IgemmArgs& a, const SpPlan& pl, hipStream_t st);
int launch_spw_kernel(const IgemmArgs& a, int wtn, int ksplit, unsigned char* img, hipStream_t st);
int launch_sp_group_kernel(int ns, const IgemmGroup& g, int wtm, int wtn, bool full, hipStream_t st);
int launch_patch_sp_kernel(int ns, const IgemmArgs& a, int wtn, int cs, int flip, int blocks, int ntotal, hipStream_t st);
int launch_sp_pgroup_kernel(int ns, const IgemmGroup& g, int wtm, int wtn, int cs, int flip, hipStream_t st);
int launch_ws_kernel(const IgemmArgs& a, int kind, int flip, int blocks, int ntotal, hipStream_t st, int ns = 4);
int launch_ws_group_kernel(const IgemmGroup& g, int flip, hipStream_t st, int ns = 4);
int launch_weight_images(const struct WeightImageGroup& g, int nblocks, hipStream_t st);
int launch_weight_image_table(const struct WeightImageTabEntry* tab, int n, int nblocks, hipStream_t st);
int launch_wgrad_sp_kernel(int ns, const WgradArgs& a, int tn, int tk, int gx, int tiles, hipStream_t st);
int launch_wgrad_group_sp(const WgradGroup& g, int tn, int tk, int nblocks, hipStream_t st);
int launch_wgrad_spw_kernel(const WgradArgs& a, int gx, int tiles, hipStream_t st);
int launch_wgrad9_kernels(int ns, int tnk, const struct Wgrad9Group& g, int nblocks, const struct Wgrad9Reduce& r, int rblocks, hipStream_t st);
int check_wgrad_span(const WgradArgs& a);
#define HRSEG_SMALL_CIN_MAX 8
void launch_small_cin_fwd(const float* x, const float* w, const float* bias, float* y, const hrseg_conv_shape_t* s, hipStream_t st);
void launch_small_cin_wgrad(const float* x, const float* dy, float* dw, const hrseg_conv_shape_t* s, int pix_per_block, hipStream_t st);
void launch_small_cin_dgrad(const float* dy, const float* w, float* dx, int accumulate, const hrseg_conv_shape_t* s, hipStream_t st);
```

### restrictive-hierarchical-semantic-segmentation_amd/csrc/conv_sp.h

```cpp
#pragma once
#include <type_traits>

typedef __bf16 bf16x8 __attribute__((ext_vector_type(8)));
typedef __bf16 bf16x2 __attribute__((ext_vector_type(2)));
typedef unsigned u32x4 __attribute__((ext_vector_type(4)));
typedef unsigned u32x2 __attribute__((ext_vector_type(2)));

__device__ __forceinline__ unsigned sp_pack_trunc(float lo, float hi) {
  return __builtin_amdgcn_perm(__float_as_uint(hi), __float_as_uint(lo), 0x07060302u);
}
__device__ __forceinline__ unsigned sp_pack_rne(float lo, float hi) {
  const bf16x2 v = {(__bf16)lo, (__bf16)hi};
  return __builtin_bit_cast(unsigned, v);
}
__device__ __forceinline__ float sp_trunc(float x) { return __uint_as_float(__float_as_uint(x) & 0xFFFF0000u); }

constexpr int sp_np(int ns) { return ns == 4 ? 2 : ns; }
constexpr int sp_products(int ns) { return ns == 1 ? 1 : ns == 3 ? 6 : 3; }
typedef _Float16 f16x8 __attribute__((ext_vector_type(8)));
typedef _Float16 f16x2 __attribute__((ext_vector_type(2)));

__device__ __forceinline__ void sp_pow2_scale(const float* absmax, float& scale, float& inv) {
  scale = inv = 1.f;
  if (!absmax) return;
// ... 258 lines not shown
      __syncthreads();
    }
  }

  const bool split = ks_n > 1;
  float* yrows[WTM];
  f32x4 add[WTM][WTN];
#pragma unroll
  for (int n = 0; n < WTN; ++n) {
    f32x4 bv = f32x4{0.f, 0.f, 0.f, 0.f};
    if (p.bias && ks_idx == 0) bv = *reinterpret_cast<const f32x4*>(p.bias + n0 + 16 * n + 4 * g);
#pragma unroll
    for (int m = 0; m < WTM; ++m) add[m][n] = bv;
  }
#pragma unroll
  for (int m = 0; m < WTM; ++m) {
    const int row = m0 + wave * 16 * WTM + 16 * m + r16;
    yrows[m] = nullptr;
    if (row >= p.M) continue;
    size_t pix = row;
    if (!p.direct_out) {
      const int b = fdiv(row, hw, p.rcp_hw);
      const int rem = row - b * hw;
      const int oy = fdiv(rem, p.Wo, p.rcp_w), ox = rem - oy * p.Wo;
      pix = (size_t)(b * p.Hy + oy * p.oys + p.oy0) * p.Wy + ox * p.oxs + p.ox0;
    }
    yrows[m] = p.y + pix * p.ldy;
    if (p.accumulate && !split) {
#pragma unroll
      for (int n = 0; n < WTN; ++n) add[m][n] += *reinterpret_cast<const f32x4*>(yrows[m] + n0 + 16 * n + 4 * g);
    }
    if (p.res && !split) {
#pragma unroll
      for (int n = 0; n < WTN; ++n) add[m][n] += *reinterpret_cast<const f32x4*>(p.res + pix * p.ldr + n0 + 16 * n + 4 * g);
    }
  }
#pragma unroll
  for (int m = 0; m < WTM; ++m) {
    float* yrow = yrows[m];
    if (!yrow) continue;
#pragma unroll
    for (int n = 0; n < WTN; ++n) {
      const int ch = n0 + 16 * n + 4 * g;
      f32x4 v = acc[n][m];
      if (NS == 4) v *= oscale;
      v += add[m][n];
      if (split) {
#pragma unroll
        for (int e = 0; e < 4; ++e) atomicAdd(yrow + ch + e, v[e]);
      } else {
        if (p.relu) {
#pragma unroll
          for (int e = 0; e < 4; ++e) v[e] = fmaxf(v[e], 0.f);
        }
        *reinterpret_cast<f32x4*>(yrow + ch) = v;
      }
    }
  }
}

template <int NS, int WTM, int WTN>
__global__ __launch_bounds__(256) void igemm_sp_kernel(IgemmArgs p) {
  __shared__ __attribute__((aligned(16))) unsigned char lds[SpLds<NS, WTN>::BYTES];
  igemm_sp_body<NS, WTM, WTN>(p, lds, blockIdx.x, gridDim.x, blockIdx.y, gridDim.y);
}

template <int NS, int WTM, int WTN, bool FULL3X3>
__global__ __launch_bounds__(256) void igemm_sp_group_kernel(IgemmGroup grp) {
  __shared__ __attribute__((aligned(16))) unsigned char lds[SpLds<NS, WTN>::BYTES];
  int gi = 0;
  while (gi + 1 < grp.n && (int)blockIdx.x >= grp.blk_end[gi]) ++gi;
  const int local = blockIdx.x - (gi ? grp.blk_end[gi - 1] : 0);
  const int tiles = grp.tiles[gi];
  igemm_sp_body<NS, WTM, WTN>(grp.a[gi], lds, local % tiles, tiles, local / tiles, grp.ksplit[gi]);
}

template <int WTN>
struct SpwLds {
  static constexpr int BN = 16 * WTN;
  static constexpr int WPIECE = BN * 64, WSTAGE = 2 * WPIECE;
  static constexpr int BYTES = 2 * WSTAGE;
};

#ifdef HRSEG_TU_IM2COL
__global__ __launch_bounds__(256) void sp_weight_image_im2col_kernel(const float* __restrict__ w, unsigned char* __restrict__ img,
                                                                     int K, int T, int ntaps, unsigned long long wtap_pk,
                                                                     float wscale, int BN, int nslabs) {
  const int slab = blockIdx.x % nslabs, nt = blockIdx.x / nslabs;
  const int kch = K >> 4, nunits = ntaps * kch;
  unsigned char* dst = img + (size_t)blockIdx.x * (size_t)(2 * BN * 64);
  for (int f = threadIdx.x; f < BN * 8; f += 256) {
    const int n = f >> 3, unit = (f >> 2) & 1, gq = f & 3;
    const int u = 2 * slab + unit;
    f32x4 v = {0.f, 0.f, 0.f, 0.f};
    if (u < nunits) {
      const int t = u / kch, c = u - t * kch;
      const int wt = (int)((wtap_pk >> (4 * t)) & 15);
      v = *reinterpret_cast<const f32x4*>(w + ((size_t)(nt * BN + n) * T + wt) * K + c * 16 + 4 * gq);
    }
    u32x2 pc[2];
    sp_split4<4>(v, pc, wscale);
    const int o = n * 64 + lds_slot(n, gq) * 16 + unit * 8;
    *reinterpret_cast<u32x2*>(dst + o) = pc[0];
    *reinterpret_cast<u32x2*>(dst + BN * 64 + o) = pc[1];
  }
}

#endif

template <int WTM, int WTN>
__device__ __forceinline__ void igemm_spw_body(const IgemmArgs& p, unsigned char* lds, const int bid, const int nblk,
                                               const int ks_idx, const int ks_n) {
  constexpr int NS = 4;
  constexpr int BM = 64 * WTM, BN = 16 * WTN;
  constexpr int WPIECE = SpwLds<WTN>::WPIECE, WSTAGE = SpwLds<WTN>::WSTAGE;
  constexpr int W16 = WSTAGE / 16;
  constexpr int W_LOADS = (W16 + 255) / 256;
  const int tid = threadIdx.x, lane = tid & 63, wave = tid >> 6;
  const int r16 = lane & 15, g = lane >> 4;
  const int ntn = p.N / BN;
  const int wg = xcd_remap(bid, nblk);
  const int nt = wg % ntn;
  const int m0 = (wg / ntn) * BM, n0 = nt * BN;

  float xscale, xinv;
  sp_pow2_scale(p.xmax, xscale, xinv);
  const float oscale = xinv * p.wscale_inv;

  const int kch = p.K >> 4;
  const int nunits = p.ntaps * kch;
  const int nslabs_all = (nunits + 1) >> 1;
  const int per = (nslabs_all + ks_n - 1) / ks_n;
  const int s_lo = ks_idx * per;
  const int s_hi = min(s_lo + per, nslabs_all);
  const int nslabs = s_hi - s_lo;

  const int hw = p.Ho * p.Wo;
  const int b0 = m0 / hw;
  const long tap0 = (long)p.oy_min * p.Wi + p.ox_min;
  const __amdgpu_buffer_rsrc_t rx = make_rsrc(p.x + ((long)b0 * p.Hi * p.Wi + tap0) * p.ldx,
                                              (size_t)((long)(p.B - b0) * p.Hi * p.Wi - tap0) * p.ldx * 4);
  const __amdgpu_buffer_rsrc_t rwi = make_rsrc(reinterpret_cast<const float*>(p.wimg), (size_t)ntn * nslabs_all * WSTAGE);

  unsigned voff[WTM];
  int inval[WTM];
#pragma unroll
  for (int m = 0; m < WTM; ++m) {
    const int row = m0 + wave * 16 * WTM + 16 * m + r16;
    if (row < p.M) {
      const int b = fdiv(row, hw, p.rcp_hw);
      const int rem = row - b * hw;
      const int oy = fdiv(rem, p.Wo, p.rcp_w), ox = rem - oy * p.Wo;
      const int iy0 = oy * p.sy, ix0 = ox * p.sx;
      voff[m] = ((unsigned)((b - b0) * p.Hi * p.Wi + iy0 * p.Wi + ix0) * (unsigned)p.ldx + 4u * g) * 4u;
      int bad = 0;
      for (int t = 0; t < p.ntaps; ++t) {
        const int iy = iy0 + (int)((p.offy_pk >> (4 * t)) & 15) - 8, ix = ix0 + (int)((p.offx_pk >> (4 * t)) & 15) - 8;
        bad |= ((iy < 0) | (iy >= p.Hi) | (ix < 0) | (ix >= p.Wi)) ? (1 << t) : 0;
      }
      inval[m] = bad;
    } else {
      voff[m] = 0;
      inval[m] = -1;
    }
  }

  constexpr int D = SP_DEPTH;
  int u_next = 2 * s_lo;
  const int u_end = min(nunits, 2 * s_hi);
  unsigned w_off = (unsigned)(nt * nslabs_all + s_lo) * (unsigned)WSTAGE;
  const unsigned w_end = (unsigned)(nt * nslabs_all + s_hi) * (unsigned)WSTAGE;
  int u_t = __builtin_amdgcn_readfirstlane(u_next / kch), u_c = u_next - u_t * kch;
  f32x4 ra[D][WTM][2], rwt[D][W_LOADS];
  auto issue_loads = [&](f32x4 (&ra)[WTM][2], f32x4 (&rwt)[W_LOADS]) {
    unsigned soff[2];
    int tapbit[2];
#pragma unroll
    for (int h = 0; h < 2; ++h) {
      const int u = u_next + h;
      const bool live = u < u_end;
      const int t = live ? u_t : 0;
      const int c = live ? u_c : 0;
      if (++u_c == kch) { u_c = 0; ++u_t; }
      const int dy = (int)((p.offy_pk >> (4 * t)) & 15) - 8 - p.oy_min, dx = (int)((p.offx_pk >> (4 * t)) & 15) - 8 - p.ox_min;
      soff[h] = live ? (unsigned)((dy * p.Wi + dx) * p.ldx + 16 * c) * 4u : 0u;
      tapbit[h] = live ? t : 31;
    }
    const bool live0 = u_next < u_end, live1 = u_next + 1 < u_end;
#pragma unroll
    for (int m = 0; m < WTM; ++m) {
#pragma unroll
      for (int h = 0; h < 2; ++h) {
        const int oob = __builtin_amdgcn_sbfe(inval[m], tapbit[h], 1) | ((h == 1 ? !live1 : !live0) ? -1 : 0);
        ra[m][h] = buf_load4(rx, voff[m] | (unsigned)oob, (int)soff[h]);
      }
    }
#pragma unroll
    for (int i = 0; i < W_LOADS; ++i) {
      const int f = tid + 256 * i;
      rwt[i] = buf_load4(rwi, (f < W16 && w_off < w_end) ? w_off + (unsigned)f * 16u : HRSEG_BUF_OOB, 0);
    }
    u_next += 2;
    w_off += WSTAGE;
  };

  constexpr int G = (WTN % 3 == 0) ? 3 : 2, NG = WTN / G;
  constexpr int MG = G * WTM * 3;
  static_assert(WTN % G == 0, "channel tiles per block: a multiple of the group size");
  constexpr int HPG = (MG - 2 * G - 2) / 4;
  static_assert(2 * NG >= W_LOADS && NG * HPG >= 2 * WTM, "a slab's MFMAs carry the whole staging of the next slab as fillers");
  unsigned xfu[2][WTM][2][4];
  f32x4 acc[WTN][WTM];
#pragma unroll
  for (int n = 0; n < WTN; ++n)
#pragma unroll
    for (int m = 0; m < WTM; ++m) acc[n][m] = f32x4{0.f, 0.f, 0.f, 0.f};

  const int foff = r16 * 64 + lds_slot(r16, g) * 16;

#pragma unroll
  for (int d = 0; d < D; ++d) issue_loads(ra[d], rwt[d]);
#pragma unroll
  for (int i = 0; i < W_LOADS; ++i) {
    const int f = tid + 256 * i;
    if (f < W16) *reinterpret_cast<f32x4*>(lds + f * 16) = rwt[0][i];
  }
#pragma unroll
  for (int m = 0; m < WTM; ++m) {
    bf16x8 t[2];
    sp_split8<NS>(ra[0][m][0], ra[0][m][1], t, xscale);
#pragma unroll
    for (int q = 0; q < 2; ++q) {
      const u32x4 u = __builtin_bit_cast(u32x4, t[q]);
#pragma unroll
      for (int e = 0; e < 4; ++e) xfu[0][m][q][e] = u[e];
    }
  }
  __syncthreads();
  auto slab = [&](auto Rc, auto Cc) {
    constexpr int R = decltype(Rc)::value, C = decltype(Cc)::value, RN = (R + 1) % D;
    issue_loads(ra[R], rwt[R]);
    const unsigned char* base = lds + C * WSTAGE;
    unsigned char* nbase = lds + (C ^ 1) * WSTAGE;
    bf16x8 wf[2][G][2];
#pragma unroll
    for (int j = 0; j < G; ++j)
#pragma unroll
      for (int q = 0; q < 2; ++q) wf[0][j][q] = *reinterpret_cast<const bf16x8*>(base + q * WPIECE + j * 1024 + foff);
    bf16x8 xcur[WTM][2];
#pragma unroll
    for (int m = 0; m < WTM; ++m)
#pragma unroll
      for (int q = 0; q < 2; ++q)
        xcur[m][q] = __builtin_bit_cast(bf16x8, (u32x4){xfu[C][m][q][0], xfu[C][m][q][1], xfu[C][m][q][2], xfu[C][m][q][3]});
    float hx[4];
    unsigned hhi[2];
#pragma unroll
    for (int k = 0; k < NG; ++k) {
#pragma unroll
      for (int pr = 0; pr < 3; ++pr)
#pragma unroll
        for (int j = 0; j < G; ++j)
#pragma unroll
          for (int m = 0; m < WTM; ++m) {
            const int i = (pr * G + j) * WTM + m;
            acc[k * G + j][m] = sp_mma_p<NS>(pr, wf[k & 1][j], xcur[m], acc[k * G + j][m]);
            if (i < 2 * G) {
              if (k + 1 < NG) {
                const int jj = i >> 1, q = i & 1;
                wf[(k + 1) & 1][jj][q] = *reinterpret_cast<const bf16x8*>(base + q * WPIECE + ((k + 1) * G + jj) * 1024 + foff);
              }
            } else if (i < 2 * G + 2) {
              const int n = 2 * k + (i - 2 * G);
              if (n < W_LOADS) {
                const int f = tid + 256 * n;
                asm volatile("" : "+v"(rwt[RN][n]));
                if (f < W16) *reinterpret_cast<f32x4*>(nbase + f * 16) = rwt[RN][n];
              }
            } else if (i < 2 * G + 2 + 4 * HPG && k * HPG + (i - (2 * G + 2)) / 4 < 2 * WTM) {
              const int h = k * HPG + (i - (2 * G + 2)) / 4;
              const int hm = h >> 1, hu = h & 1, st = (i - (2 * G + 2)) & 3;
              if (st == 0) {
                asm volatile("" : "+v"(ra[RN][hm][hu]));
#pragma unroll
                for (int e = 0; e < 4; ++e) hx[e] = ra[RN][hm][hu][e] * xscale;
              } else if (st == 1) {
                hhi[0] = sp_pack_f16_rtz(hx[0], hx[1]);
                hhi[1] = sp_pack_f16_rtz(hx[2], hx[3]);
              } else if (st == 2) {
                hx[0] -= sp_f16_lo(hhi[0]); hx[1] -= sp_f16_hi(hhi[0]);
                hx[2] -= sp_f16_lo(hhi[1]); hx[3] -= sp_f16_hi(hhi[1]);
              } else {
                xfu[C ^ 1][hm][0][2 * hu] = hhi[0];
                xfu[C ^ 1][hm][0][2 * hu + 1] = hhi[1];
                xfu[C ^ 1][hm][1][2 * hu] = sp_pack_f16_rne(hx[0], hx[1]);
                xfu[C ^ 1][hm][1][2 * hu + 1] = sp_pack_f16_rne(hx[2], hx[3]);
              }
            }
            __builtin_amdgcn_sched_barrier(0);
          }
    }
    __syncthreads();
  };
  static_assert(D == 3, "unrolled by hand: 2 * D slabs per trip");
  for (int s0 = 0; s0 < nslabs; s0 += 6) {
    slab(std::integral_constant<int, 0>{}, std::integral_constant<int, 0>{});
    slab(std::integral_constant<int, 1>{}, std::integral_constant<int, 1>{});
    slab(std::integral_constant<int, 2>{}, std::integral_constant<int, 0>{});
    slab(std::integral_constant<int, 0>{}, std::integral_constant<int, 1>{});
    slab(std::integral_constant<int, 1>{}, std::integral_constant<int, 0>{});
    slab(std::integral_constant<int, 2>{}, std::integral_constant<int, 1>{});
  }

  const bool split = ks_n > 1;
#pragma unroll
  for (int m = 0; m < WTM; ++m) {
    const int row = m0 + wave * 16 * WTM + 16 * m + r16;
    if (row >= p.M) continue;
    size_t pix = row;
    if (!p.direct_out) {
      const int b = fdiv(row, hw, p.rcp_hw);
      const int rem = row - b * hw;
      const int oy = fdiv(rem, p.Wo, p.rcp_w), ox = rem - oy * p.Wo;
      pix = (size_t)(b * p.Hy + oy * p.oys + p.oy0) * p.Wy + ox * p.oxs + p.ox0;
    }
    float* yrow = p.y + pix * p.ldy;
#pragma unroll
    for (int n = 0; n < WTN; ++n) {
      const int ch = n0 + 16 * n + 4 * g;
      f32x4 v = acc[n][m] * oscale;
      if (p.bias && ks_idx == 0) v += *reinterpret_cast<const f32x4*>(p.bias + ch);
      if (split) {
#pragma unroll
        for (int e = 0; e < 4; ++e) atomicAdd(yrow + ch + e, v[e]);
      } else {
        if (p.accumulate) v += *reinterpret_cast<const f32x4*>(yrow + ch);
        if (p.res) v += *reinterpret_cast<const f32x4*>(p.res + pix * p.ldr + ch);
        if (p.relu) {
#pragma unroll
          for (int e = 0; e < 4; ++e) v[e] = fmaxf(v[e], 0.f);
        }
        *reinterpret_cast<f32x4*>(yrow + ch) = v;
      }
    }
  }
}

template <int WTM, int WTN>
__global__ __launch_bounds__(256) void igemm_spw_kernel(IgemmArgs p) {
  __shared__ __attribute__((aligned(16))) unsigned char lds[SpwLds<WTN>::BYTES];
  igemm_spw_body<WTM, WTN>(p, lds, blockIdx.x, gridDim.x, blockIdx.y, gridDim.y);
}

typedef short s16x4 __attribute__((ext_vector_type(4)));
typedef short s16x8 __attribute__((ext_vector_type(8)));

__device__ __forceinline__ s16x4 sp_tr_read(const unsigned char* p) {
  return __builtin_amdgcn_ds_read_tr16_b64_v4i16((s16x4 __attribute__((address_space(3)))*)(p));
}

constexpr int sp_row_stride(int channels) {
  int s = (2 * channels + 31) / 32;
  if (s % 2 == 0) ++s;
  return 32 * s;
}

template <int NS, int TN, int TK>
struct SpWgradLds {
  static constexpr int PIX = 128;
  static constexpr int SA = sp_row_stride(16 * TN), SB = sp_row_stride(16 * TK);
  static constexpr int PIECE = PIX * (SA + SB);
  static constexpr int STAGE = sp_np(NS) * PIECE;
  static constexpr int RED = 4 * TK * 256 * 4;
  static constexpr int BYTES = (STAGE > RED) ? STAGE : RED;
};

template <int NS, int TN, int TK>
__device__ __forceinline__ void wgrad_sp_body(const WgradArgs& p, unsigned char* lds, const int bx, int id) {
  using L = SpWgradLds<NS, TN, TK>;
  constexpr int PIX = L::PIX, SA = L::SA, SB = L::SB, PIECE = L::PIECE;
  constexpr int ROWS = PIX / 64;
  const int tid = threadIdx.x, lane = tid & 63, wave = tid >> 6;
  const int nct = p.Cout / (16 * TN), nkt = p.Cin / (16 * TK);
  const int kt = id % nkt;
  id /= nkt;
  const int ct = id % nct;
  const int tap = id / nct;
  const int n0 = ct * 16 * TN, k0 = kt * 16 * TK;
  const int pad = (p.ks - 1) / 2;
  const int kh = tap / p.ks - pad, kw = tap % p.ks - pad;

  const int lo = bx * p.pix_per_block;
  const int hi = min(lo + p.pix_per_block, p.M);
  const int nstages = (hi - lo + PIX - 1) / PIX;
  const int q = tid & 3, r0 = tid >> 2;
  float dyscale, dyinv;
  sp_pow2_scale(p.dymax, dyscale, dyinv);

  const int hw = p.Ho * p.Wo;
  const int b_lo = lo / hw;
  const __amdgpu_buffer_rsrc_t rdy = make_rsrc(p.dy + (size_t)lo * p.lddy, (size_t)max(hi - lo, 0) * p.lddy * 4);
  const __amdgpu_buffer_rsrc_t rx =
      make_rsrc(p.x + (size_t)b_lo * p.Hi * p.Wi * p.ldx, (size_t)(p.B - b_lo) * p.Hi * p.Wi * p.ldx * 4);

  f32x4 ra[ROWS][TN], rb[ROWS][TK];
  auto stage_load = [&](int s) {
#pragma unroll
    for (int i = 0; i < ROWS; ++i) {
      const int ml = s * PIX + r0 + 64 * i;
      const int m = lo + ml;
      const bool ok = m < hi;
      const unsigned dyo = ok ? ((unsigned)ml * (unsigned)p.lddy + (unsigned)(n0 + 4 * q)) * 4u : HRSEG_BUF_OOB;
#pragma unroll
      for (int j = 0; j < TN; ++j) ra[i][j] = buf_load4(rdy, dyo, 64 * j);
      const int b = fdiv(m, hw, p.rcp_hw);
      const int rem = m - b * hw;
      const int oy = fdiv(rem, p.Wo, p.rcp_w), ox = rem - oy * p.Wo;
      const int iy = oy * p.stride + kh, ix = ox * p.stride + kw;
      const bool okx = ok & (iy >= 0) & (iy < p.Hi) & (ix >= 0) & (ix < p.Wi);
      const unsigned xo =
          okx ? ((unsigned)(((b - b_lo) * p.Hi + iy) * p.Wi + ix) * (unsigned)p.ldx + (unsigned)(k0 + 4 * q)) * 4u
              : HRSEG_BUF_OOB;
#pragma unroll
      for (int j = 0; j < TK; ++j) rb[i][j] = buf_load4(rx, xo, 64 * j);
    }
  };
  auto stage_store = [&]() {
#pragma unroll
    for (int i = 0; i < ROWS; ++i) {
      const int r = r0 + 64 * i;
#pragma unroll
      for (int j = 0; j < TN; ++j) {
        u32x2 pc[sp_np(NS)];
        sp_split4<NS>(ra[i][j], pc, dyscale);
// ... 16 lines not shown
  for (int n = 0; n < TN; ++n)
#pragma unroll
    for (int k = 0; k < TK; ++k) acc[n][k] = f32x4{0.f, 0.f, 0.f, 0.f};

  const int g = lane >> 4, li = lane & 15;
  const int prow = wave * 32 + 4 * g + (li >> 2);
  const int aoff = prow * SA + (li & 3) * 8, boff = PIX * SA + prow * SB + (li & 3) * 8;

  if (nstages > 0) {
    stage_load(0);
    stage_store();
  }
  __syncthreads();
  for (int s = 0; s < nstages; ++s) {
    const bool more = s + 1 < nstages;
    if (more) stage_load(s + 1);
    bf16x8 bfr[TK][sp_np(NS)];
#pragma unroll
    for (int k = 0; k < TK; ++k)
#pragma unroll
      for (int pc = 0; pc < sp_np(NS); ++pc) {
        const s16x4 v0 = sp_tr_read(lds + pc * PIECE + boff + k * 32);
        const s16x4 v1 = sp_tr_read(lds + pc * PIECE + boff + k * 32 + 16 * SB);
        bfr[k][pc] = __builtin_bit_cast(bf16x8, (s16x8){v0[0], v0[1], v0[2], v0[3], v1[0], v1[1], v1[2], v1[3]});
      }
#pragma unroll
    for (int n = 0; n < TN; ++n) {
      bf16x8 afr[sp_np(NS)];
#pragma unroll
      for (int pc = 0; pc < sp_np(NS); ++pc) {
        const s16x4 v0 = sp_tr_read(lds + pc * PIECE + aoff + n * 32);
        const s16x4 v1 = sp_tr_read(lds + pc * PIECE + aoff + n * 32 + 16 * SA);
        afr[pc] = __builtin_bit_cast(bf16x8, (s16x8){v0[0], v0[1], v0[2], v0[3], v1[0], v1[1], v1[2], v1[3]});
      }
#pragma unroll
      for (int pr = 0; pr < sp_nprod(NS); ++pr)
#pragma unroll
        for (int k = 0; k < TK; ++k) acc[n][k] = sp_mma_p<NS>(pr, afr, bfr[k], acc[n][k]);
    }
    __syncthreads();
    if (more) stage_store();
    __syncthreads();
  }

  float* red = reinterpret_cast<float*>(lds);
  const int r = tid >> 6, l = tid & 63;
#pragma unroll
  for (int n = 0; n < TN; ++n) {
#pragma unroll
    for (int k = 0; k < TK; ++k)
#pragma unroll
      for (int e = 0; e < 4; ++e) red[(wave * TK + k) * 256 + e * 64 + lane] = acc[n][k][e];
    __syncthreads();
#pragma unroll
    for (int k = 0; k < TK; ++k) {
      float v = 0.f;
#pragma unroll
      for (int wv = 0; wv < 4; ++wv) v += red[(wv * TK + k) * 256 + tid];
      const int co = n0 + 16 * n + 4 * (l >> 4) + r;
      const int ci = k0 + 16 * k + (l & 15);
      atomicAdd(p.dw + ((size_t)co * p.T + tap) * p.Cin + ci, NS == 4 ? v * dyinv : v);
    }
    __syncthreads();
  }
}

template <int NS, int TN, int TK>
__global__ __launch_bounds__(256) void wgrad_sp_kernel(WgradArgs p) {
  __shared__ __attribute__((aligned(16))) unsigned char lds[SpWgradLds<NS, TN, TK>::BYTES];
  const int tiles = gridDim.y, nblk = gridDim.x * gridDim.y;
  const int r = xcd_remap(blockIdx.y * gridDim.x + blockIdx.x, nblk);
  wgrad_sp_body<NS, TN, TK>(p, lds, r / tiles, r % tiles);
}

template <int NS, int TN, int TK, int NWR, int NWC>
struct SpWgradWideLds {
  static constexpr int PIX = 32;
  static constexpr int CA = 16 * TN * NWR, CB = 16 * TK * NWC;
  static constexpr int SA = sp_row_stride(CA), SB = sp_row_stride(CB);
  static constexpr int PIECE = PIX * (SA + SB);
  static constexpr int BYTES = sp_np(NS) * PIECE;
};

template <int NS, int TN, int TK, int NWR, int NWC>
__device__ __forceinline__ void wgrad_spw_body(const WgradArgs& p, unsigned char* lds, const int bx, int id) {
  using L = SpWgradWideLds<NS, TN, TK, NWR, NWC>;
  constexpr int PIX = L::PIX, SA = L::SA, SB = L::SB, PIECE = L::PIECE, CA = L::CA, CB = L::CB;
  constexpr int NT = 64 * NWR * NWC;
  constexpr int QA = CA / 4, QB = CB / 4;
  constexpr int LA = (PIX * QA + NT - 1) / NT, LB = (PIX * QB + NT - 1) / NT;
  const int tid = threadIdx.x, lane = tid & 63, wave = tid >> 6;
  const int wr = wave / NWC, wc = wave % NWC;
  const int nct = p.Cout / CA, nkt = p.Cin / CB;
  const int kt = id % nkt;
  id /= nkt;
  const int ct = id % nct;
  const int tap = id / nct;
  const int n0 = ct * CA, k0 = kt * CB;
  const int pad = (p.ks - 1) / 2;
  const int kh = tap / p.ks - pad, kw = tap % p.ks - pad;
  const int lo = bx * p.pix_per_block;
  const int hi = min(lo + p.pix_per_block, p.M);
  const int nstages = (hi - lo + PIX - 1) / PIX;
  float dyscale, dyinv;
  sp_pow2_scale(p.dymax, dyscale, dyinv);
  const int hw = p.Ho * p.Wo;
  const int b_lo = lo / hw;
  const __amdgpu_buffer_rsrc_t rdy = make_rsrc(p.dy + (size_t)lo * p.lddy, (size_t)max(hi - lo, 0) * p.lddy * 4);
  const __amdgpu_buffer_rsrc_t rx =
      make_rsrc(p.x + (size_t)b_lo * p.Hi * p.Wi * p.ldx, (size_t)(p.B - b_lo) * p.Hi * p.Wi * p.ldx * 4);

  f32x4 ra[LA], rb[LB];
  auto stage_load = [&](int s) {
#pragma unroll
    for (int i = 0; i < LA; ++i) {
      const int u = tid + NT * i, r = u / QA, cq = u - r * QA;
      const int ml = s * PIX + r;
      const bool ok = (u < PIX * QA) & (lo + ml < hi);
      ra[i] = buf_load4(rdy, ok ? ((unsigned)ml * (unsigned)p.lddy + (unsigned)(n0 + 4 * cq)) * 4u : HRSEG_BUF_OOB, 0);
    }
#pragma unroll
    for (int i = 0; i < LB; ++i) {
      const int u = tid + NT * i, r = u / QB, cq = u - r * QB;
      const int m = lo + s * PIX + r;
      const int b = fdiv(m, hw, p.rcp_hw);
      const int rem = m - b * hw;
      const int oy = fdiv(rem, p.Wo, p.rcp_w), ox = rem - oy * p.Wo;
      const int iy = oy * p.stride + kh, ix = ox * p.stride + kw;
      const bool ok = (u < PIX * QB) & (m < hi) & (iy >= 0) & (iy < p.Hi) & (ix >= 0) & (ix < p.Wi);
      rb[i] = buf_load4(rx, ok ? ((unsigned)(((b - b_lo) * p.Hi + iy) * p.Wi + ix) * (unsigned)p.ldx + (unsigned)(k0 + 4 * cq)) * 4u
                               : HRSEG_BUF_OOB, 0);
    }
  };
  auto stage_store = [&]() {
#pragma unroll
    for (int i = 0; i < LA; ++i) {
      const int u = tid + NT * i, r = u / QA, cq = u - r * QA;
      u32x2 pc[sp_np(NS)];
      sp_split4<NS>(ra[i], pc, dyscale);
      if (u < PIX * QA)
#pragma unroll
        for (int q = 0; q < sp_np(NS); ++q) *reinterpret_cast<u32x2*>(lds + q * PIECE + r * SA + cq * 8) = pc[q];
    }
#pragma unroll
    for (int i = 0; i < LB; ++i) {
      const int u = tid + NT * i, r = u / QB, cq = u - r * QB;
      u32x2 pc[sp_np(NS)];
      sp_split4<NS>(rb[i], pc);
      if (u < PIX * QB)
#pragma unroll
        for (int q = 0; q < sp_np(NS); ++q) *reinterpret_cast<u32x2*>(lds + q * PIECE + PIX * SA + r * SB + cq * 8) = pc[q];
    }
  };

  f32x4 acc[TN][TK];
#pragma unroll
  for (int n = 0; n < TN; ++n)
#pragma unroll
    for (int k = 0; k < TK; ++k) acc[n][k] = f32x4{0.f, 0.f, 0.f, 0.f};

  const int g = lane >> 4, li = lane & 15;
  const int prow = 4 * g + (li >> 2);
  const int aoff = prow * SA + (li & 3) * 8 + wr * TN * 32, boff = PIX * SA + prow * SB + (li & 3) * 8 + wc * TK * 32;

  if (nstages > 0) {
    stage_load(0);
    stage_store();
  }
  __syncthreads();
  for (int s = 0; s < nstages; ++s) {
    const bool more = s + 1 < nstages;
    if (more) stage_load(s + 1);
    bf16x8 afr[TN][sp_np(NS)];
#pragma unroll
    for (int n = 0; n < TN; ++n)
#pragma unroll
      for (int pc = 0; pc < sp_np(NS); ++pc) {
        const s16x4 v0 = sp_tr_read(lds + pc * PIECE + aoff + n * 32);
        const s16x4 v1 = sp_tr_read(lds + pc * PIECE + aoff + n * 32 + 16 * SA);
        afr[n][pc] = __builtin_bit_cast(bf16x8, (s16x8){v0[0], v0[1], v0[2], v0[3], v1[0], v1[1], v1[2], v1[3]});
      }
#pragma unroll
    for (int k = 0; k < TK; ++k) {
      bf16x8 bfr[sp_np(NS)];
#pragma unroll
      for (int pc = 0; pc < sp_np(NS); ++pc) {
        const s16x4 v0 = sp_tr_read(lds + pc * PIECE + boff + k * 32);
        const s16x4 v1 = sp_tr_read(lds + pc * PIECE + boff + k * 32 + 16 * SB);
        bfr[pc] = __builtin_bit_cast(bf16x8, (s16x8){v0[0], v0[1], v0[2], v0[3], v1[0], v1[1], v1[2], v1[3]});
      }
#pragma unroll
      for (int pr = 0; pr < sp_nprod(NS); ++pr)
#pragma unroll
        for (int n = 0; n < TN; ++n) acc[n][k] = sp_mma_p<NS>(pr, afr[n], bfr, acc[n][k]);
    }
    __syncthreads();
    if (more) stage_store();
    __syncthreads();
  }

#pragma unroll
  for (int n = 0; n < TN; ++n)
#pragma unroll
    for (int k = 0; k < TK; ++k)
#pragma unroll
      for (int e = 0; e < 4; ++e) {
        const int co = n0 + (wr * TN + n) * 16 + 4 * g + e;
        const int ci = k0 + (wc * TK + k) * 16 + li;
        atomicAdd(p.dw + ((size_t)co * p.T + tap) * p.Cin + ci, NS == 4 ? acc[n][k][e] * dyinv : acc[n][k][e]);
      }
}

template <int NS, int TN, int TK, int NWR, int NWC>
__global__ __launch_bounds__(64 * NWR * NWC) void wgrad_spw_kernel(WgradArgs p) {
  __shared__ __attribute__((aligned(16))) unsigned char lds[SpWgradWideLds<NS, TN, TK, NWR, NWC>::BYTES];
  const int tiles = gridDim.y, nblk = gridDim.x * gridDim.y;
  const int r = xcd_remap(blockIdx.y * gridDim.x + blockIdx.x, nblk);
  wgrad_spw_body<NS, TN, TK, NWR, NWC>(p, lds, r / tiles, r % tiles);
}

template <int NS, int TN, int TK>
__global__ __launch_bounds__(256) void wgrad_sp_group_kernel(WgradGroup grp) {
  __shared__ __attribute__((aligned(16))) unsigned char lds[SpWgradLds<NS, TN, TK>::BYTES];
  int g = 0;
  while (g + 1 < grp.n && (int)blockIdx.x >= grp.blk_end[g]) ++g;
  const int lo = g ? grp.blk_end[g - 1] : 0;
  const int nblk = grp.blk_end[g] - lo;
  const int tiles = nblk / grp.gx[g];
  const int r = xcd_remap(blockIdx.x - lo, nblk);
  wgrad_sp_body<NS, TN, TK>(grp.a[g], lds, r / tiles, r % tiles);
}

template <int NS, int TH, int WTN, int CS>
struct SpPatchLds {
  static constexpr int PP = (TH + 2) * 18;
  static constexpr int CHUNK = PP * 32 + ((64 - (PP * 32) % 256) + 256) % 256;
  static constexpr int PPIECE = CS * CHUNK;
  static constexpr int PATCH = sp_np(NS) * PPIECE;
  static constexpr int WPIECE = 16 * WTN * 64, WSTAGE = sp_np(NS) * WPIECE;
  static constexpr int BYTES = PATCH + 3 * WSTAGE;
};

template <int NS, int TH, int WTN, int CS, int FLIP>
__device__ __forceinline__ void igemm_patch_sp_body(const IgemmArgs& p, unsigned char* lds, const int first, const int stride,
                                                    const int end) {
  using L = SpPatchLds<NS, TH, WTN, CS>;
  constexpr int RPW = TH / 4, BN = 16 * WTN, PW = 18, PP = L::PP;
  constexpr int PG = PP * CS * 4;
  constexpr int P_LOADS = (PG + 255) / 256;
  constexpr int WG = BN * 8, W_LOADS = (WG + 255) / 256;
  constexpr int NU = 9 * CS, NSLAB = (NU + 1) / 2;
  static_assert(NSLAB % 2 == 0, "register-set parity must restart with every K stage");
  static_assert(WG >= 256 && PG >= 256, "the spare lanes of a partial round repeat a granule of the round before");
  unsigned char* lpatch = lds;
  unsigned char* lw = lds + L::PATCH;
  const int tid = threadIdx.x, lane = tid & 63, wave = tid >> 6;
  const int r16 = lane & 15, g = lane >> 4;
  const int H = p.Ho, W = p.Wo;
  const int tiles_x = (W + 15) >> 4, tiles_y = (H + TH - 1) / TH;
  const int ntn = p.N / BN;
  const int nks = p.K / (16 * CS);
  if (first >= end) return;
  const __amdgpu_buffer_rsrc_t rw = make_rsrc(p.w, (size_t)p.N * p.T * p.K * 4);
  float xscale, xinv;
  sp_pow2_scale(p.xmax, xscale, xinv);
  const float oscale = xinv * p.wscale_inv;

  struct Geom { int b, y0, x0, n0; };
  auto tile_geom = [&](int t) {
    Geom q;
    const int nt = t % ntn;
    int mt = t / ntn;
    const int tx = mt % tiles_x;
    mt /= tiles_x;
    const int ty = mt % tiles_y;
    q.b = mt / tiles_y;
    q.y0 = ty * TH; q.x0 = tx * 16; q.n0 = nt * BN;
    return q;
  };

  f32x4 rp[P_LOADS];
  auto patch_load = [&](const Geom& q, int ks) {
    const __amdgpu_buffer_rsrc_t rx = make_rsrc(p.x + (size_t)q.b * H * W * p.ldx, (size_t)H * W * p.ldx * 4);
#pragma unroll
    for (int i = 0; i < P_LOADS; ++i) {
      int f = tid + 256 * i;
      if (f >= PG) f -= 256;
      const int pix = f / (CS * 4), rem = f - pix * (CS * 4);
      const int py = pix / PW, px = pix - py * PW;
      const int iy = q.y0 - 1 + py, ix = q.x0 - 1 + px;
      const bool ok = (iy >= 0) & (iy < H) & (ix >= 0) & (ix < W);
      const unsigned off = ok ? (unsigned)(iy * W + ix) * (unsigned)(p.ldx * 4) + (unsigned)(rem * 16) : HRSEG_BUF_OOB;
      rp[i] = buf_load4(rx, off, ks * CS * 64);
    }
  };
  auto patch_store = [&]() {
#pragma unroll
    for (int i = 0; i < P_LOADS; ++i) {
      u32x2 pc[sp_np(NS)];
      sp_split4<NS>(rp[i], pc, xscale);
      int f = tid + 256 * i;
// ... 1163 lines not shown
```

### restrictive-hierarchical-semantic-segmentation_amd/csrc/conv_sp_im2col.hip

```cpp
#define HRSEG_TU_IM2COL
#include "conv_common.h"
#include "conv_sp.h"


template <int NS>
static int launch_sp(const IgemmArgs& a, const SpPlan& pl, hipStream_t st) {
#define SP2(M_, N_) \
  if (pl.wtm == M_ && pl.wtn == N_) { \
    hipLaunchKernelGGL((igemm_sp_kernel<NS, M_, N_>), dim3(ceil_div(a.M, 64 * M_) * (a.N / (16 * N_)), pl.ksplit), dim3(256), 0, st, a); \
    return 0; }
#define SP1(M_) SP2(M_, 1) SP2(M_, 2) SP2(M_, 3) SP2(M_, 4) SP2(M_, 6)
  SP1(1) SP1(2) SP1(4)
#undef SP1
#undef SP2
  return 1;
}
int launch_sp_kernel(int ns, const IgemmArgs& a, const SpPlan& pl, hipStream_t st) {
  return ns == 4 ? launch_sp<4>(a, pl, st) : ns == 3 ? launch_sp<3>(a, pl, st) : ns == 2 ? launch_sp<2>(a, pl, st) : launch_sp<1>(a, pl, st);
}

template <int NS>
static int launch_sp_group(const IgemmGroup& g, int wtm, int wtn, bool full, hipStream_t st) {
  const dim3 grid(g.blk_end[g.n - 1]);
#define SPG(M_, N_) \
  if (wtm == M_ && wtn == N_) { \
    if (full) hipLaunchKernelGGL((igemm_sp_group_kernel<NS, M_, N_, true>), grid, dim3(256), 0, st, g); \
    else hipLaunchKernelGGL((igemm_sp_group_kernel<NS, M_, N_, false>), grid, dim3(256), 0, st, g); \
    return 0; }
  SPG(1, 3) SPG(1, 4) SPG(1, 6) SPG(2, 3) SPG(2, 4) SPG(2, 6)
#undef SPG
  return 1;
}
int launch_sp_group_kernel(int ns, const IgemmGroup& g, int wtm, int wtn, bool full, hipStream_t st) {
  return ns == 4 ? launch_sp_group<4>(g, wtm, wtn, full, st) : ns == 3 ? launch_sp_group<3>(g, wtm, wtn, full, st)
       : ns == 2 ? launch_sp_group<2>(g, wtm, wtn, full, st) : launch_sp_group<1>(g, wtm, wtn, full, st);
}

int launch_spw_kernel(const IgemmArgs& a, int wtn, int ksplit, unsigned char* img, hipStream_t st) {
  const int BN = 16 * wtn;
  const int nslabs = (a.ntaps * (a.K / 16) + 1) / 2;
  hipLaunchKernelGGL(sp_weight_image_im2col_kernel, dim3((a.N / BN) * nslabs), dim3(256), 0, st, a.w, img, a.K, a.T, a.ntaps,
                     a.wtap_pk, a.wscale, BN, nslabs);
  IgemmArgs b = a;
  b.wimg = img;
  const dim3 grid(ceil_div(a.M, 128) * (a.N / BN), ksplit);
#define SPW(N_) if (wtn == N_) { hipLaunchKernelGGL((igemm_spw_kernel<2, N_>), grid, dim3(256), 0, st, b); return 0; }
  SPW(6) SPW(8) SPW(12) SPW(15)
#undef SPW
  return 1;
}
```

### restrictive-hierarchical-semantic-segmentation_amd/csrc/conv_wgrad_sp.hip

```cpp
#define HRSEG_TU_WGRAD_SP
#include "conv_common.h"
#include "conv_sp.h"


template <int NS>
static int launch_wgrad_sp(const WgradArgs& a, int tn, int tk, int gx, int tiles, hipStream_t st) {
#define WS(TN_, TK_) if (tn == TN_ && tk == TK_) { hipLaunchKernelGGL((wgrad_sp_kernel<NS, TN_, TK_>), dim3(gx, tiles), dim3(256), 0, st, a); return 0; }
  WS(1, 1) WS(1, 2) WS(1, 3) WS(1, 4) WS(2, 1) WS(2, 2) WS(2, 3) WS(2, 4)
  WS(3, 1) WS(3, 2) WS(3, 3) WS(3, 4) WS(4, 1) WS(4, 2) WS(4, 3) WS(4, 4)
  if constexpr (NS == 4) { WS(5, 5) }
#undef WS
  return HRSEG_ERR_UNSUPPORTED;
}
int launch_wgrad_sp_kernel(int ns, const WgradArgs& a, int tn, int tk, int gx, int tiles, hipStream_t st) {
  return ns == 4 ? launch_wgrad_sp<4>(a, tn, tk, gx, tiles, st) : ns == 3 ? launch_wgrad_sp<3>(a, tn, tk, gx, tiles, st)
       : ns == 2 ? launch_wgrad_sp<2>(a, tn, tk, gx, tiles, st) : launch_wgrad_sp<1>(a, tn, tk, gx, tiles, st);
}
int launch_wgrad_spw_kernel(const WgradArgs& a, int gx, int tiles, hipStream_t st) {
  hipLaunchKernelGGL((wgrad_spw_kernel<4, 5, 3, 3, 3>), dim3(gx, tiles), dim3(576), 0, st, a);
  return 0;
}
int launch_wgrad_group_sp(const WgradGroup& g, int tn, int tk, int nblocks, hipStream_t st) {
#define WGS(TN_, TK_) if (tn == TN_ && tk == TK_) { hipLaunchKernelGGL((wgrad_sp_group_kernel<4, TN_, TK_>), dim3(nblocks), dim3(256), 0, st, g); return 0; }
  WGS(3, 3) WGS(3, 4) WGS(4, 3) WGS(4, 4)
#undef WGS
  return 1;
}
int launch_wgrad9_kernels(int ns, int tnk, const Wgrad9Group& g, int nblocks, const Wgrad9Reduce& r, int rblocks, hipStream_t st) {
#define W9(NS_) if (ns == NS_) { \
    if (tnk == 3) hipLaunchKernelGGL((wgrad9_sp_group_kernel3<NS_>), dim3(nblocks), dim3(192), 0, st, g); \
    else hipLaunchKernelGGL((wgrad9_sp_group_kernel4<NS_>), dim3(nblocks), dim3(192), 0, st, g); }
  W9(1) W9(2) W9(3) W9(4)
#undef W9
  HRSEG_LAUNCH_CHECK("wgrad9");
  hipLaunchKernelGGL(wgrad9_reduce_kernel, dim3(rblocks), dim3(256), 0, st, r);
  HRSEG_LAUNCH_CHECK("wgrad9_reduce");
  return 0;
}
```

### restrictive-hierarchical-semantic-segmentation_amd/engine.py

```python
from __future__ import annotations

import contextlib
import os

import torch

from . import _lib, ops

_SIDE = {}


_SIDE_ENABLED = None
_RELU_MASK = os.environ.get("HRSEG_BN_RELU_MASK", "1") != "0"
_EXPERIMENT = set(filter(None, os.environ.get("HRSEG_EXPERIMENT", "").split(",")))
_CONV_STATS = os.environ.get("HRSEG_CONV_STATS", "1") != "0"
_X_SPLIT = int(os.environ.get("HRSEG_X_SPLIT", "2"))


def wgrad_stream(device):
    global _SIDE_ENABLED
    if _SIDE_ENABLED is None:
        _SIDE_ENABLED = os.environ.get("HRSEG_WGRAD_STREAM", "1") != "0"
    if not _SIDE_ENABLED:
        return None
    s = _SIDE.get(device)
    if s is None:
        s = _SIDE[device] = torch.cuda.Stream(device=device)
    return s


class Act:
    __slots__ = ("data", "grad", "needs_grad", "slot", "split")

    def __init__(self, data, needs_grad=True, split=False):
        self.data = data
        self.grad = None
        self.needs_grad = needs_grad
        self.split = split

    @property
    def shape(self):
        return self.data.shape


class FlatParams:

    def __init__(self, module, device):
        self.device = device
        params = [(n, p) for n, p in module.named_parameters()]
        sizes = [p.numel() for _, p in params]
        offs, total = [], 0
        for s in sizes:
            offs.append(total)
            total += (s + 3) // 4 * 4
        self.numel = total
        self.data = torch.zeros(total, dtype=torch.float32, device=device)
        self.grad = torch.zeros(total, dtype=torch.float32, device=device)
        self.slots = {}
        self.params = []
        with torch.no_grad():
            for (name, p), off, n in zip(params, offs, sizes):
                store = self.data[off:off + n]
                gstore = self.grad[off:off + n]
                if p.dim() == 4:
                    o, i, kh, kw = p.shape
                    store.view(o, kh, kw, i).copy_(p.detach().permute(0, 2, 3, 1).to(device))
                    view = store.view(o, kh, kw, i).permute(0, 3, 1, 2)
                    gview = gstore.view(o, kh, kw, i).permute(0, 3, 1, 2)
                else:
                    store.view(p.shape).copy_(p.detach().to(device))
                    view, gview = store.view(p.shape), gstore.view(p.shape)
                p.data = view
                p._hr_store, p._hr_gstore, p._hr_gview = store, gstore, gview
                p._hr_range = (off, off + n)
                self.slots[name] = (off, n)
                self.params.append(p)
        self._first, self._last = self.params[0], self.params[-1]
        self.grads_fresh = True
        import numpy as np
        entries = []
        for (name, p), off in zip(params, offs):
            if p.dim() != 4:
                continue
            o, i, kh, kw = p.shape
            if i % 16 or o % 16:
                continue
            for t in range(kh * kw):
                for co0 in range(0, o, 32):
                    for ci0 in range(0, i, 32):
                        entries.append((off, o, kh * kw, i, co0, ci0, t, 0))
            p._hr_tstore_range = (off, off + p.numel())
        self.data_t = torch.empty_like(self.data)
        self._wt_table = torch.from_numpy(np.asarray(entries, dtype=np.int32).reshape(-1)).to(device) if entries else None
        self._wt_entries = len(entries)
        self.wt_stale = True

    def transpose_all(self):
        if self.wt_stale:
            if self._wt_table is not None:
# ... 243 lines not shown
                    for i, o in zip(rnd, got):
                        xs[i].grad = o
                todo = rest
        self._push(bwd)
        return zs

    def maxpool2(self, x):
        y = Act(ops.maxpool2_fwd(x.data))
        if self.record:
            def bwd():
                g = y.grad
                y.grad = None
                if x.grad is None:
                    x.grad = ops.maxpool2_bwd(x.data, g)
                else:
                    ops.maxpool2_bwd(x.data, g, dx=x.grad, accumulate=True)
            self._push(bwd)
        return y

    def up_concat(self, low, skip, align_corners=True):
        B, Hs, Ws, Cs = skip.data.shape
        _, Hl, Wl, Cl = low.data.shape
        Hr, Wr = 2 * Hl, 2 * Wl
        py, px = (Hs - Hr) // 2, (Ws - Wr) // 2
        buf = ops.empty_nhwc(B, Hs, Ws, Cs + Cl, skip.data)
        ops.copy(skip.data, buf[..., :Cs])
        ops.bilinear_fwd(low.data, buf[..., Cs:], Hr, Wr, py, px, align_corners)
        cat = Act(buf)
        if self.record:
            def bwd():
                g = cat.grad
                cat.grad = None
                if skip.grad is None:
                    skip.grad = torch.empty(skip.data.shape, dtype=torch.float32, device=g.device)
                    ops.copy(g[..., :Cs], skip.grad)
                else:
                    ops.copy(g[..., :Cs], skip.grad, accumulate=True)
                if low.grad is None:
                    low.grad = ops.bilinear_bwd(g[..., Cs:], low.data.shape, Hr, Wr, py, px, align_corners)
                else:
                    ops.bilinear_bwd(g[..., Cs:], low.data.shape, Hr, Wr, py, px, align_corners, din=low.grad,
                                     accumulate=True)
            self._push(bwd)
        return cat

    def fuse_sum(self, terms, align_corners=True):
        same = [a for a, low in terms if not low]
        lows = [a for a, low in terms if low]
        ref = same[0]
        B, H, W, Cn = ref.data.shape
        if len(same) <= 4 and len(lows) <= 3:
            out = ops.fuse_sum([a.data for a in same], [a.data for a in lows], relu=True, align_corners=align_corners)
        else:
            if len(same) >= 2:
                out = ops.add(same[0].data, same[1].data, relu=(len(same) == 2 and not lows))
                for i, a in enumerate(same[2:]):
                    ops.add(out, a.data, relu=(i == len(same) - 3 and not lows), out=out)
            else:
                out = torch.empty(ref.data.shape, dtype=torch.float32, device=ref.data.device)
                ops.copy(ref.data, out)
            for i, a in enumerate(lows):
                ops.bilinear_fwd(a.data, out, H, W, 0, 0, align_corners, accumulate=True, relu=(i == len(lows) - 1))
        y = Act(out)
        if self.record:
            def bwd():
                g = ops.relu_bwd(y.grad, y.data, out=y.grad)
                y.grad = None
                for a in lows:
                    if a.grad is None:
                        a.grad = ops.bilinear_bwd(g, a.data.shape, H, W, 0, 0, align_corners)
                    else:
                        ops.bilinear_bwd(g, a.data.shape, H, W, 0, 0, align_corners, din=a.grad, accumulate=True)
                for i, a in enumerate(same):
                    if a.grad is not None:
                        ops.copy(g, a.grad, accumulate=True)
                    elif i == len(same) - 1:
                        a.grad = g
                    else:
                        a.grad = torch.empty(g.shape, dtype=torch.float32, device=g.device)
                        ops.copy(g, a.grad)
            self._push(bwd)
        return y

    def upsample_concat(self, xs, align_corners=True):
        B, H, W, _ = xs[0].data.shape
        chans = [x.data.shape[3] for x in xs]
        buf = ops.empty_nhwc(B, H, W, sum(chans), xs[0].data)
        ops.copy(xs[0].data, buf[..., :chans[0]])
        off = chans[0]
        for x, c in zip(xs[1:], chans[1:]):
            ops.bilinear_fwd(x.data, buf[..., off:off + c], H, W, 0, 0, align_corners)
            off += c
        cat = Act(buf)
        if self.record:
            def bwd():
                g = cat.grad
                cat.grad = None
                o = 0
                for i, (x, c) in enumerate(zip(xs, chans)):
                    gs = g[..., o:o + c]
                    if i == 0:
                        if x.grad is None:
                            x.grad = torch.empty(x.data.shape, dtype=torch.float32, device=g.device)
                            ops.copy(gs, x.grad)
                        else:
                            ops.copy(gs, x.grad, accumulate=True)
                    elif x.grad is None:
                        x.grad = ops.bilinear_bwd(gs, x.data.shape, H, W, 0, 0, align_corners)
                    else:
                        ops.bilinear_bwd(gs, x.data.shape, H, W, 0, 0, align_corners, din=x.grad, accumulate=True)
                    o += c
            self._push(bwd)
        return cat
```

### restrictive-hierarchical-semantic-segmentation_amd/ops.py

```python
from __future__ import annotations

import ctypes as C
import os

import torch

from . import _lib
from ._lib import ConvShape, call, ptr


def _ld(t):
    assert t.dim() == 4 and (t.stride(3) == 1 or t.shape[3] == 1), "NHWC tensor with contiguous channels expected"
    B, H, W, Cn = t.shape
    if W > 1:
        ld = t.stride(2)
    elif H > 1:
        ld = t.stride(1)
    elif B > 1:
        ld = t.stride(0)
    else:
        ld = Cn
    assert (H == 1 or t.stride(1) == W * ld) and (B == 1 or t.stride(0) == H * W * ld) and ld >= Cn, \
        "only channel-sliced NHWC views are supported"
    return ld
# ... 309 lines not shown
        else:
            a.partial, a.nchunks = None, 0
            outs.append((z, coef, None))
    if sync is not None:
        import torch.distributed as dist
        call("hrseg_bn_fwd_group_phases", n, arr, 1, 1)
        dist.all_reduce(pool, op=dist.ReduceOp.SUM, group=sync)
        call("hrseg_bn_fwd_group_phases", n, arr, 1, 6)
    elif phases != 7:
        call("hrseg_bn_fwd_group_phases", n, arr, int(training), int(phases))
    else:
        call("hrseg_bn_fwd_group", n, arr, int(training))
    return [(z, coef) for z, coef, _ in outs]


def bn_bwd_group(items, eval_mode, sync=None):
    n = len(items)
    arr = (_lib.BnBwd * n)()
    keep = []
    sync = None if eval_mode else sync
    ranks = _sync_world(sync) if sync is not None else 1
    pool, pool_off = None, 0
    if sync is not None:
        total = 0
        for it in items:
            Cn, npix, nseg = it["y"].shape[3], _npix(it["y"]), int(it.get("nseg", 1))
            nch = _nchunks(npix, Cn)
            nch = max(nseg, nch // nseg * nseg) if nseg > 1 else nch
            total += (nch + nseg) * 2 * Cn
        pool = zeros((total,), torch.float64, items[0]["y"].device)
    for i, (a, it) in enumerate(zip(arr, items)):
        y, dz, z = it["y"], it["dz"], it["z"]
        Cn, npix = y.shape[3], _npix(y)
        nseg = int(it.get("nseg", 1))
        nch = _nchunks(npix, Cn)
        if nseg > 1:
            nch = max(nseg, nch // nseg * nseg)
        if pool is not None:
            part = pool[pool_off:pool_off + (nch + nseg) * 2 * Cn]
            pool_off += (nch + nseg) * 2 * Cn
        else:
            part = torch.empty((nch + nseg) * 2 * Cn, dtype=torch.float64, device=y.device)
        keep.append(part)
        a.nseg = nseg
        a.sum_ranks = ranks
        dres = it.get("dres")
        a.dz, a.lddz = ptr(dz), _ld(dz)
        use_z = it["relu"] and z is not None
        a.z, a.ldz, a.relu = (ptr(z) if use_z else None), (_ld(z) if use_z else 0), int(it["relu"])
        a.y, a.ldy, a.coef = ptr(y), _ld(y), ptr(it["coef"])
        a.dgamma, a.dbeta = ptr(it["dgamma"]), ptr(it["dbeta"])
        a.dy, a.lddy = ptr(dz), _ld(dz)
        a.dres, a.lddres = ptr(dres), (_ld(dres) if dres is not None else 0)
        a.dres_accumulate = int(bool(it.get("dres_accumulate", False)))
        a.npix, a.C, a.partial, a.nchunks = npix, Cn, ptr(part), nch
        a.dy_absmax = ptr(it.get("dy_absmax"))
        a.relu_mask = ptr(it.get("relu_mask"))
    if sync is not None:
        import torch.distributed as dist
        call("hrseg_bn_bwd_group_phases", n, arr, 0, 1)
        dist.all_reduce(pool, op=dist.ReduceOp.SUM, group=sync)
        call("hrseg_bn_bwd_group_phases", n, arr, 0, 6)
    else:
        call("hrseg_bn_bwd_group", n, arr, int(eval_mode))
    return [it["dz"] for it in items]


def maxpool2_fwd(x):
    B, H, W, Cn = x.shape
    y = empty_nhwc(B, H // 2, W // 2, Cn, x)
    call("hrseg_maxpool2_fwd", ptr(x), _ld(x), ptr(y), _ld(y), B, H, W, Cn)
    return y


def maxpool2_bwd(x, dy, dx=None, accumulate=False):
    B, H, W, Cn = x.shape
    if dx is None:
        dx = torch.empty(x.shape, dtype=torch.float32, device=x.device)
        accumulate = False
    call("hrseg_maxpool2_bwd", ptr(x), _ld(x), ptr(dy), _ld(dy), ptr(dx), _ld(dx), int(accumulate), B, H, W, Cn)
    return dx


def bilinear_fwd(x, out, Hr, Wr, py=0, px=0, align_corners=True, accumulate=False, relu=False):
    B, Hi, Wi, Cn = x.shape
    call("hrseg_bilinear_fwd", ptr(x), _ld(x), B, Hi, Wi, Cn, ptr(out), _ld(out), out.shape[1], out.shape[2], Hr, Wr,
         py, px, int(align_corners), int(accumulate), int(relu))
    return out


def bilinear_bwd(dout, x_shape, Hr, Wr, py=0, px=0, align_corners=True, din=None, accumulate=False):
    B, Hi, Wi, Cn = x_shape
    if din is None:
        din = empty_nhwc(B, Hi, Wi, Cn, dout)
        accumulate = False
    call("hrseg_bilinear_bwd", ptr(dout), _ld(dout), B, Hi, Wi, Cn, ptr(din), _ld(din), dout.shape[1], dout.shape[2],
         Hr, Wr, py, px, int(align_corners), int(accumulate))
    return din


def fuse_sum(same, lows, relu=True, align_corners=True):
    ref = same[0]
    B, H, W, Cn = ref.shape
    out = torch.empty(ref.shape, dtype=torch.float32, device=ref.device)
    call("hrseg_fuse_sum", len(same), _lib.ptr_array(same), _lib.int_array([_ld(t) for t in same]), len(lows),
         _lib.ptr_array(lows) if lows else None, _lib.int_array([_ld(t) for t in lows]) if lows else None,
         _lib.int_array([t.shape[1] for t in lows]) if lows else None, _lib.int_array([t.shape[2] for t in lows]) if lows else None,
         ptr(out), _ld(out), B, H, W, Cn, int(align_corners), int(relu))
    return out


def add(a, b, relu=False, out=None):
    if out is None:
        out = torch.empty(a.shape, dtype=torch.float32, device=a.device)
    call("hrseg_add", ptr(a), _ld(a), ptr(b), _ld(b), ptr(out), _ld(out), int(relu), _npix(a), a.shape[3])
    return out


def copy(src, dst, accumulate=False):
    call("hrseg_copy", ptr(src), _ld(src), ptr(dst), _ld(dst), int(accumulate), _npix(src), src.shape[3])
    return dst


def relu_bwd(dz, z, out=None):
    if out is None:
        out = torch.empty(z.shape, dtype=torch.float32, device=z.device)
    call("hrseg_relu_bwd", ptr(dz), _ld(dz), ptr(z), _ld(z), ptr(out), _ld(out), _npix(z), z.shape[3])
    return out


def nchw_to_nhwc(x, out=None):
    B, Cn, H, W = x.shape
    if out is None:
        out = empty_nhwc(B, H, W, Cn, x)
    call("hrseg_nchw_to_nhwc", ptr(x), ptr(out), Cn, B, Cn, H, W)
    return out


def nhwc_to_nchw(x):
    B, H, W, Cn = x.shape
    out = torch.empty((B, Cn, H, W), dtype=torch.float32, device=x.device)
    call("hrseg_nhwc_to_nchw", ptr(x), _ld(x), ptr(out), B, Cn, H, W)
    return out


def concat_image_logits(x, z):
    x, z = _c(x.float()), _c(z.float())
    B, Ci, H, W = x.shape
    Cz = z.shape[1]
    out = torch.empty((B, H, W, Ci + Cz), dtype=torch.float32, device=x.device)
    call("hrseg_nchw_to_nhwc", ptr(x), ptr(out), Ci + Cz, B, Ci, H, W)
    call("hrseg_nchw_to_nhwc", ptr(z), out.data_ptr() + 4 * Ci, Ci + Cz, B, Cz, H, W)
    return out


def nhwc_slice_to_nchw(g, c0):
    B, H, W, Cn = g.shape
    assert g.is_contiguous()
    out = torch.empty((B, Cn - c0, H, W), dtype=torch.float32, device=g.device)
    call("hrseg_nhwc_to_nchw", g.data_ptr() + 4 * c0, Cn, ptr(out), B, Cn - c0, H, W)
    return out


def accumulate_flat(dst, src):
    n = dst.numel()
    assert src.numel() == n and dst.is_contiguous() and src.is_contiguous()
    if n % 4 == 0 and n > 0:
        call("hrseg_copy", ptr(src), 4, ptr(dst), 4, 1, n // 4, 4)
    else:
        dst.add_(src)
    return dst


def encode_targets(label, on_lut, parent):
    assert label.dtype == torch.uint8 and label.is_cuda and label.dim() == 3
    assert on_lut.dtype == torch.int64 and on_lut.numel() == 256 and on_lut.is_cuda
    label = label.contiguous()
    B, H, W = label.shape
    Cn = len(parent)
    out = torch.empty((B, Cn, H, W), dtype=torch.float32, device=label.device)
    call("hrseg_encode_targets", ptr(label), ptr(on_lut), _lib.int_array(list(parent)), ptr(out), B, Cn, H * W)
    return out


def augment_workspace(B, S):
    img, tgt = C.c_size_t(0), C.c_size_t(0)
    _lib.call_raw("hrseg_augment_workspace", int(B), int(S), C.byref(img), C.byref(tgt))
    return int(img.value), int(tgt.value)


def _check_ragged(buf, desc, desc_host, channels):
    assert buf.dtype == torch.uint8 and buf.is_cuda and buf.dim() == 1 and buf.is_contiguous()
    assert desc.dtype == torch.int64 and desc.is_cuda and desc.shape == desc_host.shape and desc.dim() == 2 and desc.shape[1] == 4
    n = buf.numel()
    for off, H, W, ch in desc_host.tolist():
        if ch not in channels or H < 1 or W < 1 or off < 0 or off + H * W * ch > n:
            raise ValueError(f"ragged descriptor (offset {off}, {H}x{W}, {ch} channels) does not fit a {n}-byte buffer")


def augment_image(src, desc, desc_host, params, S, train):
    _check_ragged(src, desc, desc_host, (1, 3))
    B = desc.shape[0]
    x = torch.empty((B, 3, S, S), dtype=torch.float32, device=src.device)
# ... 236 lines not shown
```

Measured before the change: 90.81 images/s.

## Pre-split shared-head concat activations to fp16x2 and add a 1x1 tap fast path

The upsample-concat that feeds the shared head conv now writes its output directly as pre-split fp16x2 pieces, fused into the copy and bilinear kernels. The wide-tile forward igemm and the wide wgrad kernel can consume these pieces without re-splitting, which removes the per-tile split work on a large activation in both forward and weight-gradient passes. A specialised single-tap load path is also added for 1x1 convs in the wide kernel. The change adds template variants and routing checks, and every other consumer of the concat buffer, such as the concat backward, must handle the split format correctly.

```diff
diff --git a/restrictive-hierarchical-semantic-segmentation_amd/Models/models.py b/restrictive-hierarchical-semantic-segmentation_amd/Models/models.py
--- a/restrictive-hierarchical-semantic-segmentation_amd/Models/models.py
+++ b/restrictive-hierarchical-semantic-segmentation_amd/Models/models.py
@@ -758,7 +758,7 @@
             for mod in getattr(self, f"stage{t_idx + 1}"):
                 ys = mod.run(rec, ys)
         rec.mark("shared_head")
-        cat = rec.upsample_concat(ys, self.align_corners)
+        cat = rec.upsample_concat(ys, self.align_corners, split_for=self.shared_head[0])
         return rec.conv_bn(cat, self.shared_head[0], self.shared_head[1], relu=True)
 
     def forward(self, x):
diff --git a/restrictive-hierarchical-semantic-segmentation_amd/csrc/bn_elem.hip b/restrictive-hierarchical-semantic-segmentation_amd/csrc/bn_elem.hip
--- a/restrictive-hierarchical-semantic-segmentation_amd/csrc/bn_elem.hip
+++ b/restrictive-hierarchical-semantic-segmentation_amd/csrc/bn_elem.hip
@@ -367,12 +367,13 @@
       v = ly0 * (lx0 * v00 + lx1 * v01) + ly1 * (lx0 * v10 + lx1 * v11);
     }
     float* o = out + pix * ldout + 4 * L.cq;
-    if (acc) v += ld4(o);
+    if (acc == 1) v += ld4(o);
     if (relu) {
 #pragma unroll
       for (int j = 0; j < 4; ++j) v[j] = fmaxf(v[j], 0.f);
     }
-    st4(o, v);
+    if (acc == 2) *reinterpret_cast<hrseg_u32x4*>(o) = hrseg_split_f16x2(v);
+    else st4(o, v);
   }
 }
 
@@ -501,7 +502,8 @@
   FOR_PIXELS(pix, L, npix) {
     f32x4 v = ld4(in + pix * ldin + 4 * L.cq);
     float* o = out + pix * ldout + 4 * L.cq;
-    st4(o, acc ? ld4(o) + v : v);
+    if (acc == 2) *reinterpret_cast<hrseg_u32x4*>(o) = hrseg_split_f16x2(v);
+    else st4(o, acc ? ld4(o) + v : v);
   }
 }
 __global__ __launch_bounds__(256) void relu_bwd_kernel(const float* __restrict__ dz, int lddz,
@@ -1004,6 +1006,7 @@
   HRSEG_CHECK_ARG(in && out && B > 0 && Hi > 0 && Wi > 0 && Hr > 0 && Wr > 0 && py >= 0 && px >= 0 &&
                       py + Hr <= Hout && px + Wr <= Wout,
                   "hrseg_bilinear_fwd: placed image %dx%d at (%d,%d) does not fit %dx%d", Hr, Wr, py, px, Hout, Wout);
+  HRSEG_CHECK_ARG(accumulate >= 0 && accumulate <= 2, "hrseg_bilinear_fwd: accumulate %d (0 store, 1 add, 2 store pre-split)", accumulate);
   const long npix = (long)B * Hout * Wout;
   hipLaunchKernelGGL(bilinear_fwd_kernel, dim3(elem_grid(npix, C)), dim3(256), 0, (hipStream_t)stream, in, ldin, B, Hi,
                      Wi, C, out, ldout, Hout, Wout, Hr, Wr, py, px, resize_scale(Hi, Hr, align_corners),
@@ -1076,7 +1079,7 @@
 extern "C" int hrseg_copy(const float* in, int ldin, float* out, int ldout, int accumulate, long npix, int C,
                           hrseg_stream_t stream) {
   if (int e = check_c(C, "hrseg_copy")) return e;
-  HRSEG_CHECK_ARG(in && out && npix > 0, "hrseg_copy: bad arguments");
+  HRSEG_CHECK_ARG(in && out && npix > 0 && accumulate >= 0 && accumulate <= 2, "hrseg_copy: bad arguments");
   hipLaunchKernelGGL(copy_kernel, dim3(elem_grid(npix, C)), dim3(256), 0, (hipStream_t)stream, in, ldin, out, ldout,
                      accumulate, npix, C);
   HRSEG_LAUNCH_CHECK("copy");
diff --git a/restrictive-hierarchical-semantic-segmentation_amd/csrc/conv.hip b/restrictive-hierarchical-semantic-segmentation_amd/csrc/conv.hip
--- a/restrictive-hierarchical-semantic-segmentation_amd/csrc/conv.hip
+++ b/restrictive-hierarchical-semantic-segmentation_amd/csrc/conv.hip
@@ -432,6 +432,7 @@
 
 static int g_sp_wide = 1;
 static int g_spw_min_blocks = 256;
+static int g_spw_tap1 = 1;
 static int spw_wtn(const IgemmArgs& a) {
   if (!g_sp_wide || !scratch_usable() || a.K % 16 || a.M < 128) return 0;
   const int wtn = (a.N % 240 == 0) ? 15 : (a.N % 192 == 0) ? 12 : (a.N % 128 == 0) ? 8 : (a.N % 96 == 0) ? 6 : 0;
@@ -468,8 +469,14 @@
 }
 
 static int x_split_unsupported(const char* who) {
-  hrseg_set_error("%s: x_split is set but this problem does not run the wave-specialised / nine-tap kernels (ask hrseg_conv_x_split_ok first)", who);
+  hrseg_set_error("%s: x_split is set but this problem does not run the wave-specialised / nine-tap / wide-tile kernels (ask hrseg_conv_x_split_ok first)", who);
   return HRSEG_ERR_UNSUPPORTED;
+}
+static int g_x_split_wide = 1;
+static bool spw_route(const IgemmArgs& a, int ns) {
+  if (ns != 4 || g_sp_wtn) return false;
+  if (patch_cs(a, plan_sp(a).wtn)) return false;
+  return spw_wtn(a) != 0;
 }
 static int dispatch_igemm(const IgemmArgs& a_in, int precision, hipStream_t st) {
   IgemmArgs a = a_in;
@@ -481,7 +488,7 @@
       const int kind = ws_kind(a);
       if (kind && ws_tiles(a, kind) >= g_ws_min_tiles && launch_ws_single(a, kind, st, ns) == 0) return 0;
     }
-    if (a.x_presplit) return x_split_unsupported("hrseg_conv_fwd");
+    if (a.x_presplit && !(g_x_split_wide && spw_route(a, ns))) return x_split_unsupported("hrseg_conv_fwd");
     if (const int cs = patch_cs(a, pl.wtn)) {
       const int rc = launch_patch_sp(ns, a, pl.wtn, cs, st);
       if (rc == 0) return 0;
@@ -492,10 +499,11 @@
         const size_t bytes = (size_t)(a.N / (16 * wtn)) * ((a.ntaps * (a.K / 16) + 1) / 2) * (size_t)(2 * 16 * wtn * 64);
         if (unsigned char* img = scratch_reserve(st, bytes)) {
           ++g_cnt[CNT_SP_WIDE];
-          if (launch_spw_kernel(a, wtn, 1, img, st) == 0) return 0;
+          if (launch_spw_kernel(a, wtn, 1, img, g_spw_tap1 != 0, st) == 0) return 0;
         }
       }
     }
+    if (a.x_presplit) return x_split_unsupported("hrseg_conv_fwd");
     if (pl.ksplit > 1 && !a.accumulate) zero_f32(a.y, (size_t)a.B * a.Hy * a.Wy * a.N, st);
     return launch_sp(ns, a, pl, st);
   }
@@ -704,8 +712,12 @@
   }
   return best;
 }
+static bool wgrad_wide_route(int ns, const WgradArgs& a) {
+  return ns == 4 && g_wg_wide && a.Cout % 240 == 0 && a.Cin % 144 == 0 && a.M >= 65536 && !hrseg_g_deterministic && !g_tune_wg_blocks;
+}
 static int dispatch_wgrad_sp(int ns, WgradArgs a, hipStream_t st) {
-  if (ns == 4 && g_wg_wide && a.Cout % 240 == 0 && a.Cin % 144 == 0 && a.M >= 65536 && !hrseg_g_deterministic && !g_tune_wg_blocks) {
+  if (a.x_presplit && !wgrad_wide_route(ns, a)) return x_split_unsupported("hrseg_conv_wgrad");
+  if (wgrad_wide_route(ns, a)) {
     const int tiles = (a.Cout / 240) * (a.Cin / 144) * a.T;
     int kmax = a.M / 2048;
     if (kmax > 64) kmax = 64;
@@ -1071,8 +1083,10 @@
 }
 
 static int g_x_split = 1;
+static bool x_split_wide_ok(const hrseg_conv_shape_t& s);
 extern "C" int hrseg_conv_x_split_ok(int n, const hrseg_conv_shape_t* shapes) {
   if (!g_x_split || !shapes || n < 1 || n > MAXG || n > WG9_MAXG) return 0;
+  if (n == 1 && x_split_wide_ok(shapes[0])) return 1;
   if (!g_sp_ws || !scratch_usable() || g_sp_wtn || g_tune_wtm || g_tune_kc || g_tune_db || g_tune_ksplit) return 0;
   for (int i = 0; i < n; ++i) {
     const hrseg_conv_shape_t& s = shapes[i];
@@ -1117,6 +1131,7 @@
   hipStream_t st = (hipStream_t)stream;
   HRSEG_CHECK_ARG(s->Cout % 16 == 0 || s->Cin <= HRSEG_SMALL_CIN_MAX, "hrseg_conv_fwd: Cout %d not a multiple of 16", s->Cout);
   if (s->Cin <= HRSEG_SMALL_CIN_MAX) {
+    if (s->x_split) return x_split_unsupported("hrseg_conv_fwd");
     launch_small_cin_fwd(x, w, bias, y, s, st);
     ++g_cnt[CNT_SMALL_CIN];
     HRSEG_LAUNCH_CHECK("conv_small_cin_fwd");
@@ -1198,9 +1213,27 @@
   return 0;
 }
 
+static bool x_split_wide_ok(const hrseg_conv_shape_t& s) {
+  if (!g_x_split_wide || s.residual || s.relu || !mfma_shape(&s) || s.Cin <= HRSEG_SMALL_CIN_MAX || s.Cin % 16 || s.ldx % 4 || s.ldy % 4) return false;
+  if (check_shape(&s, "hrseg_conv_x_split_ok")) return false;
+  IgemmArgs a;
+  fill_fwd_args(a, reinterpret_cast<const float*>(256), reinterpret_cast<const float*>(256), nullptr, reinterpret_cast<float*>(256), &s);
+  a.stat_partial = nullptr; a.stat_rows = nullptr;
+  if (finalize_args(a)) return false;
+  const int ns = sp_pieces(resolve_auto(a, s.precision));
+  if (!ns) return false;
+  const int kind = ws_kind(a);
+  if ((ns == 4 || (ns == 1 && g_ws_bf16)) && !g_sp_wtn && kind && ws_tiles(a, kind) >= g_ws_min_tiles) return false;
+  if (!spw_route(a, ns)) return false;
+  hrseg_conv_shape_t r;
+  resolve_wgrad_shapes(1, &s, &r);
+  WgradArgs g;
+  fill_wgrad_args(g, reinterpret_cast<const float*>(256), reinterpret_cast<const float*>(256), reinterpret_cast<float*>(256), &r);
+  return wgrad_wide_route(sp_pieces(r.precision), g);
+}
+
 extern "C" int hrseg_conv_wgrad(const float* x, const float* dy, float* dw, const hrseg_conv_shape_t* s_in,
                                 hrseg_stream_t stream) {
-  if (s_in && s_in->x_split) return x_split_unsupported("hrseg_conv_wgrad");
   HRSEG_CHECK_ARG(s_in != nullptr, "hrseg_conv_wgrad: null shape");
   hrseg_conv_shape_t sh;
   resolve_wgrad_shapes(1, s_in, &sh);
@@ -1208,7 +1241,7 @@
   if (int e = check_shape(s, "hrseg_conv_wgrad")) return e;
   HRSEG_CHECK_ARG(x && dy && dw, "hrseg_conv_wgrad: null pointer");
   hipStream_t st = (hipStream_t)stream;
-  const int T = s->ksize * s->ksize;
+  if (s->x_split && (s->Cin <= HRSEG_SMALL_CIN_MAX || !sp_pieces(s->precision) || !g_x_split_wide)) return x_split_unsupported("hrseg_conv_wgrad");
   if (s->Cin <= HRSEG_SMALL_CIN_MAX) {
     const long M = (long)s->B * s->Ho * s->Wo;
     const int nblk_target = hrseg_g_deterministic ? 1 : g_tune_wg_blocks ? g_tune_wg_blocks : 512;
@@ -1221,15 +1254,11 @@
   HRSEG_CHECK_ARG(s->Cin % 16 == 0 && s->Cout % 16 == 0, "hrseg_conv_wgrad: channels (%d,%d) must be multiples of 16",
                   s->Cin, s->Cout);
   HRSEG_CHECK_ARG(s->ldx % 4 == 0 && s->ldy % 4 == 0, "hrseg_conv_wgrad: ld must be a multiple of 4");
-  WgradArgs a{};
-  a.x = x; a.dy = dy; a.dw = dw; a.ldx = s->ldx; a.lddy = s->ldy;
-  a.B = s->B; a.Hi = s->Hi; a.Wi = s->Wi; a.Cin = s->Cin; a.Ho = s->Ho; a.Wo = s->Wo; a.Cout = s->Cout;
-  a.M = s->B * s->Ho * s->Wo; a.ks = s->ksize; a.stride = s->stride; a.T = T;
-  const bool big = (long)s->B * s->Ho * s->Wo >= (1L << 24);
-  a.rcp_hw = big ? 0.f : 1.0f / (float)(s->Ho * s->Wo);
-  a.rcp_w = big ? 0.f : 1.0f / (float)s->Wo;
-  a.dymax = s->precision == HRSEG_CONV_FP16X2 ? s->grad_absmax : nullptr;
+  WgradArgs a;
+  fill_wgrad_args(a, x, dy, dw, s);
+  a.x_presplit = s->x_split;
   if (const int ns = sp_pieces(s->precision)) {
+    if (a.x_presplit && !wgrad_wide_route(ns, a)) return x_split_unsupported("hrseg_conv_wgrad");
     if (int e = dispatch_wgrad_sp(ns, a, st)) return e;
     HRSEG_LAUNCH_CHECK("wgrad_sp");
     return 0;
@@ -1274,7 +1303,7 @@
       {"igemm_wtm", &g_tune_wtm}, {"igemm_kc", &g_tune_kc}, {"igemm_db", &g_tune_db}, {"igemm_ksplit", &g_tune_ksplit},
       {"group_wtm", &g_group_wtm}, {"wgrad_pix", &g_tune_wg_pix}, {"wgrad_db", &g_tune_wg_db},
       {"wgrad_blocks", &g_tune_wg_blocks}, {"wgrad_group_mult", &g_wg_mult}, {"wgrad_group_min", &g_wg_min},
-      {"wgrad_group_max", &g_wg_max}, {"sp_wtm", &g_sp_wtm}, {"sp_wtn", &g_sp_wtn}, {"sp_ksplit", &g_sp_ksplit}, {"sp_patch", &g_sp_patch}, {"sp_persist", &g_sp_persist}, {"sp_ws", &g_sp_ws}, {"sp_ws_waste", &g_ws_waste}, {"small_cin3", &g_small_cin3}, {"sp_ws_bf16", &g_ws_bf16}, {"sp_ws_n48", &g_ws_n48}, {"sp_img", &g_sp_img}, {"wgrad9", &g_wg9}, {"ws_epi_early", &g_ws_epi_early}, {"exp_nosplit_x", &g_exp_nosplit}, {"x_split", &g_x_split}, {"ws_epi_cost", &g_ws_epi_cost}, {"ws_epi_acc_cost", &g_ws_epi_acc_cost}, {"wgrad9_blocks", &g_wg9_blocks}, {"wgrad9_blocks1", &g_wg9_blocks_n[1]}, {"wgrad9_blocks2", &g_wg9_blocks_n[2]}, {"wgrad9_blocks3", &g_wg9_blocks_n[3]}, {"wgrad9_blocks4", &g_wg9_blocks_n[4]}, {"sp_wide", &g_sp_wide}, {"sp_ws_canvas", &g_ws_canvas}, {"wgrad_group_sp", &g_wg_group_sp}, {"wgrad_sp_t5", &g_wg_t5}, {"wgrad_sp_wide", &g_wg_wide}, {"sp_wide_min_blocks", &g_spw_min_blocks},
+      {"wgrad_group_max", &g_wg_max}, {"sp_wtm", &g_sp_wtm}, {"sp_wtn", &g_sp_wtn}, {"sp_ksplit", &g_sp_ksplit}, {"sp_patch", &g_sp_patch}, {"sp_persist", &g_sp_persist}, {"sp_ws", &g_sp_ws}, {"sp_ws_waste", &g_ws_waste}, {"small_cin3", &g_small_cin3}, {"sp_ws_bf16", &g_ws_bf16}, {"sp_ws_n48", &g_ws_n48}, {"sp_img", &g_sp_img}, {"wgrad9", &g_wg9}, {"ws_epi_early", &g_ws_epi_early}, {"exp_nosplit_x", &g_exp_nosplit}, {"x_split", &g_x_split}, {"x_split_wide", &g_x_split_wide}, {"sp_wide_tap1", &g_spw_tap1}, {"ws_epi_cost", &g_ws_epi_cost}, {"ws_epi_acc_cost", &g_ws_epi_acc_cost}, {"wgrad9_blocks", &g_wg9_blocks}, {"wgrad9_blocks1", &g_wg9_blocks_n[1]}, {"wgrad9_blocks2", &g_wg9_blocks_n[2]}, {"wgrad9_blocks3", &g_wg9_blocks_n[3]}, {"wgrad9_blocks4", &g_wg9_blocks_n[4]}, {"sp_wide", &g_sp_wide}, {"sp_ws_canvas", &g_ws_canvas}, {"wgrad_group_sp", &g_wg_group_sp}, {"wgrad_sp_t5", &g_wg_t5}, {"wgrad_sp_wide", &g_wg_wide}, {"sp_wide_min_blocks", &g_spw_min_blocks},
       {"sp_patch_min_tiles", &g_patch_min_tiles}, {"auto_min_pixels", &g_auto_min_pix}, {"sp_ws_min_tiles", &g_ws_min_tiles},
       {"deterministic", &hrseg_g_deterministic}};
   HRSEG_CHECK_ARG(key != nullptr, "hrseg_tune: null key");
diff --git a/restrictive-hierarchical-semantic-segmentation_amd/csrc/conv_common.h b/restrictive-hierarchical-semantic-segmentation_amd/csrc/conv_common.h
--- a/restrictive-hierarchical-semantic-segmentation_amd/csrc/conv_common.h
+++ b/restrictive-hierarchical-semantic-segmentation_amd/csrc/conv_common.h
@@ -83,6 +83,7 @@
   int pix_per_block;
   float rcp_hw, rcp_w;
   const float* dymax;
+  int x_presplit;
 };
 
 struct WgradGroup {
@@ -99,7 +100,7 @@
 int launch_wgrad_f32(const WgradArgs& a, int tn, int tk, int pix, int db, int target, hipStream_t st);
 int launch_wgrad_group_f32(const WgradGroup& g, int tn, int tk, int nblocks, hipStream_t st);
 int launch_sp_kernel(int ns, const IgemmArgs& a, const SpPlan& pl, hipStream_t st);
-int launch_spw_kernel(const IgemmArgs& a, int wtn, int ksplit, unsigned char* img, hipStream_t st);
+int launch_spw_kernel(const IgemmArgs& a, int wtn, int ksplit, unsigned char* img, bool tap1, hipStream_t st);
 int launch_sp_group_kernel(int ns, const IgemmGroup& g, int wtm, int wtn, bool full, hipStream_t st);
 int launch_patch_sp_kernel(int ns, const IgemmArgs& a, int wtn, int cs, int flip, int blocks, int ntotal, hipStream_t st);
 int launch_sp_pgroup_kernel(int ns, const IgemmGroup& g, int wtm, int wtn, int cs, int flip, hipStream_t st);
diff --git a/restrictive-hierarchical-semantic-segmentation_amd/csrc/conv_sp.h b/restrictive-hierarchical-semantic-segmentation_amd/csrc/conv_sp.h
--- a/restrictive-hierarchical-semantic-segmentation_amd/csrc/conv_sp.h
+++ b/restrictive-hierarchical-semantic-segmentation_amd/csrc/conv_sp.h
@@ -364,7 +364,7 @@
   static constexpr int BYTES = 2 * WSTAGE;
 };
 
-#ifdef HRSEG_TU_IM2COL
+#ifdef HRSEG_TU_SPW
 __global__ __launch_bounds__(256) void sp_weight_image_im2col_kernel(const float* __restrict__ w, unsigned char* __restrict__ img,
                                                                      int K, int T, int ntaps, unsigned long long wtap_pk,
                                                                      float wscale, int BN, int nslabs) {
@@ -390,7 +390,7 @@
 
 #endif
 
-template <int WTM, int WTN>
+template <int WTM, int WTN, bool XS, bool TAP1>
 __device__ __forceinline__ void igemm_spw_body(const IgemmArgs& p, unsigned char* lds, const int bid, const int nblk,
                                                const int ks_idx, const int ks_n) {
   constexpr int NS = 4;
@@ -453,12 +453,25 @@
   unsigned w_off = (unsigned)(nt * nslabs_all + s_lo) * (unsigned)WSTAGE;
   const unsigned w_end = (unsigned)(nt * nslabs_all + s_hi) * (unsigned)WSTAGE;
   int u_t = __builtin_amdgcn_readfirstlane(u_next / kch), u_c = u_next - u_t * kch;
+  const unsigned tap1_off = (unsigned)((((int)(p.offy_pk & 15) - 8 - p.oy_min) * p.Wi + ((int)(p.offx_pk & 15) - 8 - p.ox_min)) * p.ldx) * 4u;
   f32x4 ra[D][WTM][2], rwt[D][W_LOADS];
+  unsigned voff1[WTM];
+#pragma unroll
+  for (int m = 0; m < WTM; ++m) voff1[m] = voff[m] | ((inval[m] & 1) ? ~0u : 0u);
   auto issue_loads = [&](f32x4 (&ra)[WTM][2], f32x4 (&rwt)[W_LOADS]) {
     unsigned soff[2];
     int tapbit[2];
-#pragma unroll
-    for (int h = 0; h < 2; ++h) {
+    if constexpr (TAP1) {
+#pragma unroll
+      for (int h = 0; h < 2; ++h) {
+        const bool live = u_next + h < u_end;
+        const unsigned dead = live ? 0u : ~0u;
+#pragma unroll
+        for (int m = 0; m < WTM; ++m) ra[m][h] = buf_load4(rx, voff1[m] | dead, live ? (int)(tap1_off + 64u * (unsigned)(u_next + h)) : 0);
+      }
+    }
+#pragma unroll
+    for (int h = 0; h < 2 && !TAP1; ++h) {
       const int u = u_next + h;
       const bool live = u < u_end;
       const int t = live ? u_t : 0;
@@ -470,7 +483,7 @@
     }
     const bool live0 = u_next < u_end, live1 = u_next + 1 < u_end;
 #pragma unroll
-    for (int m = 0; m < WTM; ++m) {
+    for (int m = 0; m < WTM && !TAP1; ++m) {
 #pragma unroll
       for (int h = 0; h < 2; ++h) {
         const int oob = __builtin_amdgcn_sbfe(inval[m], tapbit[h], 1) | ((h == 1 ? !live1 : !live0) ? -1 : 0);
@@ -509,6 +522,15 @@
   }
 #pragma unroll
   for (int m = 0; m < WTM; ++m) {
+    if (XS) {
+#pragma unroll
+      for (int h = 0; h < 2; ++h) {
+        const u32x4 u = __builtin_bit_cast(u32x4, ra[0][m][h]);
+#pragma unroll
+        for (int e = 0; e < 4; ++e) xfu[0][m][e >> 1][2 * h + (e & 1)] = u[e];
+      }
+      continue;
+    }
     bf16x8 t[2];
     sp_split8<NS>(ra[0][m][0], ra[0][m][1], t, xscale);
 #pragma unroll
@@ -562,7 +584,13 @@
             } else if (i < 2 * G + 2 + 4 * HPG && k * HPG + (i - (2 * G + 2)) / 4 < 2 * WTM) {
               const int h = k * HPG + (i - (2 * G + 2)) / 4;
               const int hm = h >> 1, hu = h & 1, st = (i - (2 * G + 2)) & 3;
-              if (st == 0) {
+              if (XS) {
+                if (st == 0) {
+                  const u32x4 u = __builtin_bit_cast(u32x4, ra[RN][hm][hu]);
+#pragma unroll
+                  for (int e = 0; e < 4; ++e) xfu[C ^ 1][hm][e >> 1][2 * hu + (e & 1)] = u[e];
+                }
+              } else if (st == 0) {
                 asm volatile("" : "+v"(ra[RN][hm][hu]));
 #pragma unroll
                 for (int e = 0; e < 4; ++e) hx[e] = ra[RN][hm][hu][e] * xscale;
@@ -628,10 +656,10 @@
   }
 }
 
-template <int WTM, int WTN>
+template <int WTM, int WTN, bool XS = false, bool TAP1 = false>
 __global__ __launch_bounds__(256) void igemm_spw_kernel(IgemmArgs p) {
   __shared__ __attribute__((aligned(16))) unsigned char lds[SpwLds<WTN>::BYTES];
-  igemm_spw_body<WTM, WTN>(p, lds, blockIdx.x, gridDim.x, blockIdx.y, gridDim.y);
+  igemm_spw_body<WTM, WTN, XS, TAP1>(p, lds, blockIdx.x, gridDim.x, blockIdx.y, gridDim.y);
 }
 
 typedef short s16x4 __attribute__((ext_vector_type(4)));
@@ -814,7 +842,7 @@
   static constexpr int BYTES = sp_np(NS) * PIECE;
 };
 
-template <int NS, int TN, int TK, int NWR, int NWC>
+template <int NS, int TN, int TK, int NWR, int NWC, bool XS>
 __device__ __forceinline__ void wgrad_spw_body(const WgradArgs& p, unsigned char* lds, const int bx, int id) {
   using L = SpWgradWideLds<NS, TN, TK, NWR, NWC>;
   constexpr int PIX = L::PIX, SA = L::SA, SB = L::SB, PIECE = L::PIECE, CA = L::CA, CB = L::CB;
@@ -878,7 +906,14 @@
     for (int i = 0; i < LB; ++i) {
       const int u = tid + NT * i, r = u / QB, cq = u - r * QB;
       u32x2 pc[sp_np(NS)];
-      sp_split4<NS>(rb[i], pc);
+      if constexpr (XS) {
+        static_assert(!XS || NS == 4, "pre-split activations are fp16x2 pieces");
+        const u32x4 v = __builtin_bit_cast(u32x4, rb[i]);
+        pc[0] = u32x2{v[0], v[1]};
+        pc[1] = u32x2{v[2], v[3]};
+      } else {
+        sp_split4<NS>(rb[i], pc);
+      }
       if (u < PIX * QB)
 #pragma unroll
         for (int q = 0; q < sp_np(NS); ++q) *reinterpret_cast<u32x2*>(lds + q * PIECE + PIX * SA + r * SB + cq * 8) = pc[q];
@@ -943,12 +978,12 @@
       }
 }
 
-template <int NS, int TN, int TK, int NWR, int NWC>
+template <int NS, int TN, int TK, int NWR, int NWC, bool XS = false>
 __global__ __launch_bounds__(64 * NWR * NWC) void wgrad_spw_kernel(WgradArgs p) {
   __shared__ __attribute__((aligned(16))) unsigned char lds[SpWgradWideLds<NS, TN, TK, NWR, NWC>::BYTES];
   const int tiles = gridDim.y, nblk = gridDim.x * gridDim.y;
   const int r = xcd_remap(blockIdx.y * gridDim.x + blockIdx.x, nblk);
-  wgrad_spw_body<NS, TN, TK, NWR, NWC>(p, lds, r / tiles, r % tiles);
+  wgrad_spw_body<NS, TN, TK, NWR, NWC, XS>(p, lds, r / tiles, r % tiles);
 }
 
 template <int NS, int TN, int TK>
diff --git a/restrictive-hierarchical-semantic-segmentation_amd/csrc/conv_sp_im2col.hip b/restrictive-hierarchical-semantic-segmentation_amd/csrc/conv_sp_im2col.hip
--- a/restrictive-hierarchical-semantic-segmentation_amd/csrc/conv_sp_im2col.hip
+++ b/restrictive-hierarchical-semantic-segmentation_amd/csrc/conv_sp_im2col.hip
@@ -35,17 +35,3 @@
   return ns == 4 ? launch_sp_group<4>(g, wtm, wtn, full, st) : ns == 3 ? launch_sp_group<3>(g, wtm, wtn, full, st)
        : ns == 2 ? launch_sp_group<2>(g, wtm, wtn, full, st) : launch_sp_group<1>(g, wtm, wtn, full, st);
 }
-
-int launch_spw_kernel(const IgemmArgs& a, int wtn, int ksplit, unsigned char* img, hipStream_t st) {
-  const int BN = 16 * wtn;
-  const int nslabs = (a.ntaps * (a.K / 16) + 1) / 2;
-  hipLaunchKernelGGL(sp_weight_image_im2col_kernel, dim3((a.N / BN) * nslabs), dim3(256), 0, st, a.w, img, a.K, a.T, a.ntaps,
-                     a.wtap_pk, a.wscale, BN, nslabs);
-  IgemmArgs b = a;
-  b.wimg = img;
-  const dim3 grid(ceil_div(a.M, 128) * (a.N / BN), ksplit);
-#define SPW(N_) if (wtn == N_) { hipLaunchKernelGGL((igemm_spw_kernel<2, N_>), grid, dim3(256), 0, st, b); return 0; }
-  SPW(6) SPW(8) SPW(12) SPW(15)
-#undef SPW
-  return 1;
-}
diff --git a/restrictive-hierarchical-semantic-segmentation_amd/csrc/conv_sp_wide.hip b/restrictive-hierarchical-semantic-segmentation_amd/csrc/conv_sp_wide.hip
--- /dev/null
+++ b/restrictive-hierarchical-semantic-segmentation_amd/csrc/conv_sp_wide.hip
@@ -0,0 +1,28 @@
+#define HRSEG_TU_SPW
+#include "conv_common.h"
+#include "conv_sp.h"
+
+template <int WTN>
+static void launch_spw(const IgemmArgs& b, dim3 grid, bool tap1, hipStream_t st) {
+  if (b.x_presplit) {
+    if (tap1) hipLaunchKernelGGL((igemm_spw_kernel<2, WTN, true, true>), grid, dim3(256), 0, st, b);
+    else hipLaunchKernelGGL((igemm_spw_kernel<2, WTN, true, false>), grid, dim3(256), 0, st, b);
+  } else {
+    if (tap1) hipLaunchKernelGGL((igemm_spw_kernel<2, WTN, false, true>), grid, dim3(256), 0, st, b);
+    else hipLaunchKernelGGL((igemm_spw_kernel<2, WTN, false, false>), grid, dim3(256), 0, st, b);
+  }
+}
+
+int launch_spw_kernel(const IgemmArgs& a, int wtn, int ksplit, unsigned char* img, bool tap1, hipStream_t st) {
+  const int BN = 16 * wtn;
+  const int nslabs = (a.ntaps * (a.K / 16) + 1) / 2;
+  hipLaunchKernelGGL(sp_weight_image_im2col_kernel, dim3((a.N / BN) * nslabs), dim3(256), 0, st, a.w, img, a.K, a.T, a.ntaps,
+                     a.wtap_pk, a.wscale, BN, nslabs);
+  IgemmArgs b = a;
+  b.wimg = img;
+  const dim3 grid(ceil_div(a.M, 128) * (a.N / BN), ksplit);
+#define SPW(N_) if (wtn == N_) { launch_spw<N_>(b, grid, tap1 && a.ntaps == 1, st); return 0; }
+  SPW(6) SPW(8) SPW(12) SPW(15)
+#undef SPW
+  return 1;
+}
diff --git a/restrictive-hierarchical-semantic-segmentation_amd/csrc/conv_wgrad_sp.hip b/restrictive-hierarchical-semantic-segmentation_amd/csrc/conv_wgrad_sp.hip
--- a/restrictive-hierarchical-semantic-segmentation_amd/csrc/conv_wgrad_sp.hip
+++ b/restrictive-hierarchical-semantic-segmentation_amd/csrc/conv_wgrad_sp.hip
@@ -17,7 +17,8 @@
        : ns == 2 ? launch_wgrad_sp<2>(a, tn, tk, gx, tiles, st) : launch_wgrad_sp<1>(a, tn, tk, gx, tiles, st);
 }
 int launch_wgrad_spw_kernel(const WgradArgs& a, int gx, int tiles, hipStream_t st) {
-  hipLaunchKernelGGL((wgrad_spw_kernel<4, 5, 3, 3, 3>), dim3(gx, tiles), dim3(576), 0, st, a);
+  if (a.x_presplit) hipLaunchKernelGGL((wgrad_spw_kernel<4, 5, 3, 3, 3, true>), dim3(gx, tiles), dim3(576), 0, st, a);
+  else hipLaunchKernelGGL((wgrad_spw_kernel<4, 5, 3, 3, 3, false>), dim3(gx, tiles), dim3(576), 0, st, a);
   return 0;
 }
 int launch_wgrad_group_sp(const WgradGroup& g, int tn, int tk, int nblocks, hipStream_t st) {
diff --git a/restrictive-hierarchical-semantic-segmentation_amd/engine.py b/restrictive-hierarchical-semantic-segmentation_amd/engine.py
--- a/restrictive-hierarchical-semantic-segmentation_amd/engine.py
+++ b/restrictive-hierarchical-semantic-segmentation_amd/engine.py
@@ -15,6 +15,7 @@
 _EXPERIMENT = set(filter(None, os.environ.get("HRSEG_EXPERIMENT", "").split(",")))
 _CONV_STATS = os.environ.get("HRSEG_CONV_STATS", "1") != "0"
 _X_SPLIT = int(os.environ.get("HRSEG_X_SPLIT", "2"))
+_X_SPLIT_WIDE = os.environ.get("HRSEG_X_SPLIT_WIDE", "1") != "0"
 
 
 def wgrad_stream(device):
@@ -424,16 +425,20 @@
             self._push(bwd)
         return y
 
-    def upsample_concat(self, xs, align_corners=True):
+    def upsample_concat(self, xs, align_corners=True, split_for=None):
         B, H, W, _ = xs[0].data.shape
         chans = [x.data.shape[3] for x in xs]
         buf = ops.empty_nhwc(B, H, W, sum(chans), xs[0].data)
-        ops.copy(xs[0].data, buf[..., :chans[0]])
+        split = False
+        if split_for is not None and _X_SPLIT_WIDE and _X_SPLIT >= 1 and not _EXPERIMENT and self.training and self.record:
+            split = ops.conv_x_split_ok([tuple(buf.shape)], [split_for.out_channels], split_for.kernel_size[0],
+                                        split_for.stride[0], self.prec)
+        ops.copy(xs[0].data, buf[..., :chans[0]], split=split)
         off = chans[0]
         for x, c in zip(xs[1:], chans[1:]):
-            ops.bilinear_fwd(x.data, buf[..., off:off + c], H, W, 0, 0, align_corners)
+            ops.bilinear_fwd(x.data, buf[..., off:off + c], H, W, 0, 0, align_corners, split=split)
             off += c
-        cat = Act(buf)
+        cat = Act(buf, split=split)
         if self.record:
             def bwd():
                 g = cat.grad
diff --git a/restrictive-hierarchical-semantic-segmentation_amd/ops.py b/restrictive-hierarchical-semantic-segmentation_amd/ops.py
--- a/restrictive-hierarchical-semantic-segmentation_amd/ops.py
+++ b/restrictive-hierarchical-semantic-segmentation_amd/ops.py
@@ -415,7 +415,9 @@
     return dx
 
 
-def bilinear_fwd(x, out, Hr, Wr, py=0, px=0, align_corners=True, accumulate=False, relu=False):
+def bilinear_fwd(x, out, Hr, Wr, py=0, px=0, align_corners=True, accumulate=False, relu=False, split=False):
+    assert not (split and accumulate)
+    accumulate = 2 if split else int(accumulate)
     B, Hi, Wi, Cn = x.shape
     call("hrseg_bilinear_fwd", ptr(x), _ld(x), B, Hi, Wi, Cn, ptr(out), _ld(out), out.shape[1], out.shape[2], Hr, Wr,
          py, px, int(align_corners), int(accumulate), int(relu))
@@ -450,8 +452,9 @@
     return out
 
 
-def copy(src, dst, accumulate=False):
-    call("hrseg_copy", ptr(src), _ld(src), ptr(dst), _ld(dst), int(accumulate), _npix(src), src.shape[3])
+def copy(src, dst, accumulate=False, split=False):
+    assert not (split and accumulate)
+    call("hrseg_copy", ptr(src), _ld(src), ptr(dst), _ld(dst), 2 if split else int(accumulate), _npix(src), src.shape[3])
     return dst
 
 
```

Result: no change. 91.03 images/s, median of 6 (+0.2%).
